# caiyuanhao1998/Open-DiffusionGS

Measured on AMD Instinct MI355X. Metric: novel-view renders/sec (DiT step + GS raster) at 256^2, higher is better.
Workload: dtype bf16; 1 GPU; obj-256 sampling step (BASELINE.json configs[2]): DGSDenoiser.forward = DiT image_to_gaussians (width 1024, 24 blocks, L=4098, bf16 MFMA, fp32 accumulate) + 4 fp32 rasterizations of P=262146 Gaussians at 256^2 per sample; random-init weights; batch_per_gpu=1, views=4, resolution=256, gaussians=262146, parallelism=dp1

## Files before the change

### include/dgs_dit.h

```cpp
#ifndef DGS_DIT_H_
#define DGS_DIT_H_

#include <stddef.h>
#include <stdint.h>

#include "dgs_raster.h"

#ifdef __cplusplus
extern "C" {
#endif

typedef enum DgsGemmEpilogue {
    DGS_EPI_BF16 = 0,
    DGS_EPI_GELU_BF16 = 1,
    DGS_EPI_GATE_RESIDUAL = 2,
    DGS_EPI_F32 = 3,
    DGS_EPI_QKV = 4,
    DGS_EPI_DGELU_BF16 = 5
} DgsGemmEpilogue;

typedef enum DgsGemmAlgo {
    DGS_GEMM_AUTO = 0,
    DGS_GEMM_SIMPLE128 = 1,
    DGS_GEMM_SLICED = 4,
    DGS_GEMM_QUAD = 5,
    DGS_GEMM_SLICED128 = 6
} DgsGemmAlgo;

typedef struct DgsDitGemmArgs {
    int32_t M, N, K;
    const uint16_t* A;
    int32_t lda;
    const uint16_t* W;
    int32_t ldw;
    const float* bias;
    int32_t epilogue;
    void* out;
    int32_t ldo;
    const float* gate;
    int32_t gate_stride;
    int32_t rows_per_batch;
    uint16_t* vt;
    const float* resid;
    void* aux;
    int32_t k_per_batch;
    int64_t a_batch_stride, w_batch_stride;
    int32_t algo;
    int32_t valid_rows;
    float q_scale;
    float* splitk_ws;
} DgsDitGemmArgs;

size_t dgs_dit_gemm_splitk_bytes(int32_t M, int32_t N, int32_t K, int32_t k_per_batch);

typedef struct DgsDitAttentionArgs {
    int32_t B, heads, L, lpad;
    const uint16_t* qk;
    const uint16_t* vt;
    uint16_t* out;
    float scale;
    int32_t ld_qk;
    int32_t k_offset;
    int64_t vt_batch_stride;
    float* lse2;
    int32_t q_prescaled;
    void* tail_ws;
    size_t tail_ws_bytes;
    int32_t tail_mode;
} DgsDitAttentionArgs;

size_t dgs_dit_attention_tail_bytes(int32_t B, int32_t heads, int32_t L);

typedef struct DgsDitAttentionBackwardArgs {
    int32_t B, heads, L, lpad;
    const uint16_t* qkv;
    const uint16_t* qkvT;
    const uint16_t* o;
    const uint16_t* dO;
    const uint16_t* dOT;
    const float* lse2;
    float* D;
    uint16_t* dqkv;
    float scale;
    uint16_t* dqkvT;
    float* bias_part;
} DgsDitAttentionBackwardArgs;
int32_t dgs_dit_attention_backward_slots(int32_t L);

typedef struct DgsDitLayerNormArgs {
    int32_t rows, width;
    const float* x;
    const float* weight;
    const float* shift;
    const float* scale;
    int32_t mod_stride;
    int32_t rows_per_batch;
    float eps;
    void* out;
    int32_t out_f32;
} DgsDitLayerNormArgs;

typedef struct DgsDitLayerNormBackwardArgs {
    int32_t rows, width;
    const float* x;
    const void* dh;
    int32_t dh_f32;
    const float* weight;
    const float* scale;
    int32_t mod_stride, rows_per_batch;
    float eps;
    const float* dx_in;
    float* dx_out;
    float *dshift, *dscale, *dweight;
    void* scratch;
    size_t scratch_bytes;
} DgsDitLayerNormBackwardArgs;

typedef struct DgsDitRowLinearBackwardArgs {
    int32_t M, N, K;
    const float* x;
    int32_t silu_input;
    const uint16_t* W;
    const float* dy;
    float *dW, *db, *dx;
    void* scratch;
    size_t scratch_bytes;
} DgsDitRowLinearBackwardArgs;

typedef struct DgsDitGateMulArgs {
    int32_t B, rows, width;
    const float* dx;
    const uint16_t* y;
    const float* gate;
    int32_t gate_stride;
    uint16_t *dy, *dyT;
    float* dgate;
    float* dbias;
    void* scratch;
    size_t scratch_bytes;
} DgsDitGateMulArgs;

typedef struct DgsDitRowLinearArgs {
    int32_t M, N, K;
    const float* x;
    int32_t silu_input;
    const uint16_t* W;
    const float* bias;
    int32_t silu_output;
    float* out;
} DgsDitRowLinearArgs;

typedef struct DgsDitLayerWeights {
    const uint16_t *qkv_w, *proj_w, *fc1_w, *fc2_w;
    const float *qkv_b, *proj_b, *fc1_b, *fc2_b;
} DgsDitLayerWeights;

typedef struct DgsDitModel {
    int32_t width, heads, layers, patch, in_channels, n_gaussians, gs_channels;
    int32_t scene;
    int32_t relative_plk;
    float range_near, range_far;
    const uint16_t* t_w0; const float* t_b0;
    const uint16_t* t_w1; const float* t_b1;
    const uint16_t* tok_w;
    const float* pos_emb;
    const float* in_ln_w;
    const DgsDitLayerWeights* layer;
    const uint16_t* ada_w; const float* ada_b;
    const float* up_ln_w;  const uint16_t* up_w;
    const float* dec_ln_w; const uint16_t* dec_w;
} DgsDitModel;

typedef struct DgsDitForwardArgs {
    int32_t B, V, H, W;
    const float* images;
    const float* ray_o;
    const float* ray_d;
    const int64_t* t;
    void* workspace;
    size_t workspace_bytes;
    float* xyz;
    float* features;
    float* scaling;
    float* rotation;
    float* opacity;
    float* aligned_xyz;
    float* tokens;
    void** prof_events;
    int32_t prof_kind;
    int32_t prof_capacity;
    int32_t* prof_count;
    int32_t train_recompute;
} DgsDitForwardArgs;

typedef struct DgsDitLayerWeightsT {
    const uint16_t *qkv_wT, *proj_wT, *fc1_wT, *fc2_wT;
} DgsDitLayerWeightsT;

typedef struct DgsDitModelT {
    const DgsDitLayerWeightsT* layer;
    const uint16_t* dec_wT;
} DgsDitModelT;

typedef struct DgsDitLayerGrads {
    float *qkv_w, *proj_w, *fc1_w, *fc2_w, *qkv_b, *proj_b, *fc1_b, *fc2_b;
    float *ada_w, *ada_b;
} DgsDitLayerGrads;

typedef struct DgsDitGrads {
    float *t_w0, *t_b0, *t_w1, *t_b1, *tok_w, *pos_emb, *in_ln_w;
    const DgsDitLayerGrads* layer;
    float *head_ada_w, *head_ada_b;
    float *up_ln_w, *up_w, *dec_ln_w, *dec_w;
} DgsDitGrads;

typedef struct DgsDitBackwardArgs {
    int32_t B, V, H, W;
    const float* ray_d;
    void* saved;        size_t saved_bytes;
    void* workspace;    size_t workspace_bytes;
    const float *dxyz, *dfeatures, *dscaling, *drotation, *dopacity;
    int32_t recompute;
    void (*block_done)(void* user, int32_t stage);
    void* block_user;
} DgsDitBackwardArgs;

size_t dgs_dit_saved_bytes(const DgsDitModel* m, int32_t B, int32_t V, int32_t H, int32_t W, int32_t recompute);
size_t dgs_dit_backward_workspace_bytes(const DgsDitModel* m, int32_t B, int32_t V, int32_t H, int32_t W);
int dgs_dit_forward_train(const DgsDitModel* m, const DgsDitForwardArgs* a, void* saved, size_t saved_bytes, dgs_stream_t stream);
int dgs_dit_backward(const DgsDitModel* m, const DgsDitModelT* mt, const DgsDitGrads* grads, const DgsDitBackwardArgs* a,
                     dgs_stream_t stream);

int dgs_dit_gemm(const DgsDitGemmArgs* a, dgs_stream_t stream);
int32_t dgs_dit_gemm_sliced_tile(const DgsDitGemmArgs* a);
int dgs_dit_attention(const DgsDitAttentionArgs* a, dgs_stream_t stream);
int dgs_dit_attention_backward(const DgsDitAttentionBackwardArgs* a, dgs_stream_t stream);
int dgs_dit_layernorm(const DgsDitLayerNormArgs* a, dgs_stream_t stream);
int dgs_dit_layernorm_gemm(const DgsDitLayerNormArgs* ln, const DgsDitGemmArgs* g, dgs_stream_t stream);
int32_t dgs_dit_layernorm_gemm_shares_rows(const DgsDitLayerNormArgs* ln, const DgsDitGemmArgs* g);
int dgs_dit_layernorm_backward(const DgsDitLayerNormBackwardArgs* a, dgs_stream_t stream);
int dgs_dit_rowlinear_backward(const DgsDitRowLinearBackwardArgs* a, dgs_stream_t stream);
int dgs_dit_gate_mul(const DgsDitGateMulArgs* a, dgs_stream_t stream);
size_t dgs_dit_layernorm_backward_scratch_bytes(int32_t rows, int32_t width, int32_t rows_per_batch);
size_t dgs_dit_rowlinear_backward_scratch_bytes(int32_t M, int32_t N, int32_t K);
size_t dgs_dit_gate_mul_scratch_bytes(int32_t B, int32_t rows, int32_t width);
int dgs_dit_rowlinear(const DgsDitRowLinearArgs* a, dgs_stream_t stream);

typedef struct DgsDitRunBlocksArgs {
    int32_t B, L, V;
    int32_t first, last;
    const float* tokens_in;
    const float* cvec;
    float* tokens_out;
    void* workspace;
    size_t workspace_bytes;
} DgsDitRunBlocksArgs;
size_t dgs_dit_workspace_bytes_for_tokens(const DgsDitModel* m, int32_t B, int32_t L);
int dgs_dit_run_blocks(const DgsDitModel* m, const DgsDitRunBlocksArgs* a, dgs_stream_t stream);

int dgs_debug_poison_lds(dgs_stream_t stream);

int dgs_debug_clock_probe(int64_t* out, int32_t microseconds, dgs_stream_t stream);

int32_t dgs_dit_lpad(int32_t L);
size_t dgs_dit_workspace_bytes(const DgsDitModel* m, int32_t B, int32_t V, int32_t H, int32_t W);
int dgs_dit_forward(const DgsDitModel* m, const DgsDitForwardArgs* a, dgs_stream_t stream);

#ifdef __cplusplus
}
#endif
#endif
```

### open-diffusiongs_amd/csrc/dit_gemm.hip

```cpp
#include <stdlib.h>

#include "dit_common.h"
#include "dgs_dit.h"
#include "dit_gemm_epilogue.h"

namespace dgs {

constexpr int BM = 128, BK = 64;
constexpr int TILE_BYTES = BM * BK * 2;

struct GemmParams {
    int M, N, K, lda, ldw, ldo, gate_stride, rows_per_batch, valid_rows, tiles_n, ntiles, tiles_m, map_mode;
    int rows_ps, full_rows;
    int ntail, tail_row0;
    int k_per_batch;
    long long a_batch_stride, w_batch_stride;
    const bf16_t* A;
    const bf16_t* W;
    const float* bias;
    void* out;
    const float* gate;
    const float* resid;
    bf16_t* vt;
    void* aux;
    float q_scale;
};

__device__ __forceinline__ float gelu_tanh(float x) {
    const float u = 0.7978845608028654f * (x + 0.044715f * x * x * x);
    return x / (1.0f + __expf(-2.0f * u));
}

__device__ __forceinline__ float dgelu_tanh(float x) {
    const float u = 0.7978845608028654f * (x + 0.044715f * x * x * x);
    const float sg = 1.0f / (1.0f + __expf(-2.0f * u));
    return sg + x * sg * (1.0f - sg) * (2.0f * 0.7978845608028654f) * (1.0f + 3.0f * 0.044715f * x * x);
}

template <int ROWS>
__device__ __forceinline__ void stage_tile(const bf16_t* g, int ld, int row0, int k0, char* lds_tile, int wave, int lane) {
#pragma unroll
    for (int q = 0; q < ROWS / 32; ++q) {
        const int piece = wave * (ROWS / 32) + q;
        const int row = piece * 8 + (lane >> 3);
        const int slot = lane & 7;
        const int chunk = slot ^ ((row >> 1) & 7);
        const bf16_t* src = g + (size_t)(row0 + row) * ld + k0 + chunk * 8;
        glds16(src, lds_tile + piece * 1024);
    }
}

template <int NI, int MI>
__device__ __forceinline__ void mma_tile(const char* la, const char* lb, int fhalf, int swz, f32x16 (&acc)[2][NI]) {
    bf16x8 a[2][MI], b[2][NI];
    auto read = [&](int ks, int h) {
        const int off = ((2 * ks + fhalf) ^ swz) << 4;
#pragma unroll
        for (int i = 0; i < MI; ++i) a[h][i] = *reinterpret_cast<const bf16x8*>(la + i * 32 * 128 + off);
#pragma unroll
        for (int j = 0; j < NI; ++j) b[h][j] = *reinterpret_cast<const bf16x8*>(lb + j * 32 * 128 + off);
    };
    read(0, 0);
#pragma unroll
    for (int ks = 0; ks < 4; ++ks) {
        const int h = ks & 1;
#pragma unroll
        for (int i = 0; i < MI; ++i)
#pragma unroll
            for (int j = 0; j < NI; ++j) {
                acc[i][j] = __builtin_amdgcn_mfma_f32_32x32x16_bf16(a[h][i], b[h][j], acc[i][j], 0, 0, 0);
                if (i == 0 && j == 0 && ks < 3) read(ks + 1, h ^ 1);
                sched_fence();
            }
    }
}

template <int BN, int NI, int MI, bool ONE_BATCH>
__device__ __forceinline__ void main_loop(const GemmParams& p, char* lds, int m0, int n0, int wave, int lane, int wm, int wn,
                                          f32x16 (&acc)[2][NI]) {
    constexpr int STAGE_BYTES = TILE_BYTES + BN * BK * 2;
    const int nk = p.K / BK;
    const int spb = p.k_per_batch / BK;
    stage_tile<BM>(p.A, p.lda, m0, 0, lds, wave, lane);
    stage_tile<BN>(p.W, p.ldw, n0, 0, lds + TILE_BYTES, wave, lane);
    __syncthreads();
    const int frow = lane & 31, fhalf = lane >> 5;
    const int swz = (frow >> 1) & 7;
    for (int t = 0; t < nk; ++t) {
        char* cur = lds + (t & 1) * STAGE_BYTES;
        if (t + 1 < nk) {
            char* nxt = lds + ((t + 1) & 1) * STAGE_BYTES;
            const int bb = ONE_BATCH ? 0 : (t + 1) / spb, kk = ((t + 1) - bb * spb) * BK;
            stage_tile<BM>(p.A + bb * p.a_batch_stride, p.lda, m0, kk, nxt, wave, lane);
            stage_tile<BN>(p.W + bb * p.w_batch_stride, p.ldw, n0, kk, nxt + TILE_BYTES, wave, lane);
        }
        if (MI > 0) {
            const char* la = cur + (wm * 64 + frow) * 128;
            const char* lb = cur + TILE_BYTES + (wn * (BN / 2) + frow) * 128;
            mma_tile<NI, (MI > 0 ? MI : 1)>(la, lb, fhalf, swz, acc);
        }
        __syncthreads();
    }
}

template <int EPI>
__device__ __forceinline__ void gemv_tail_rows(const GemmParams& p, char* lds, int item, int wave, int lane) {
    constexpr int CPI = 8;
    const int nblk = p.N / CPI, b = item / nblk, tn0 = (item - b * nblk) * CPI;
    const int tm0 = b * p.rows_per_batch + p.tail_row0;
    const int kw = p.K / 4, k_lo = wave * kw;
    const int nch = (kw + 511) / 512;
    const bool on0 = lane * 8 < kw, on1 = 512 + lane * 8 < kw;
    const bf16_t* a_row0 = p.A + (size_t)tm0 * p.lda + k_lo + lane * 8;
    const bf16_t* w_col0 = p.W + (size_t)tn0 * p.ldw + k_lo + lane * 8;
    const uint4 zero = make_uint4(0u, 0u, 0u, 0u);
    const int er = lane / CPI, ec = lane - er * CPI;
    const bool finisher = wave == 0 && lane < 2 * CPI && p.tail_row0 + er < p.valid_rows;
    TailOperands ops{0.f, 0.f, 0.f};
    if (finisher) ops = tail_prefetch<EPI>(p, tm0 + er, tn0 + ec);
    uint4 a[2][2], w[CPI][2];
#pragma unroll
    for (int ch = 0; ch < 2; ++ch) {
        const bool on = ch == 0 ? on0 : (on1 && nch > 1);
#pragma unroll
        for (int r = 0; r < 2; ++r) a[r][ch] = on ? *reinterpret_cast<const uint4*>(a_row0 + (size_t)r * p.lda + ch * 512) : zero;
#pragma unroll
        for (int c = 0; c < CPI; ++c) w[c][ch] = on ? *reinterpret_cast<const uint4*>(w_col0 + (size_t)c * p.ldw + ch * 512) : zero;
    }
    float* const part = reinterpret_cast<float*>(lds);
#pragma unroll
    for (int c = 0; c < CPI; ++c) {
        float s0 = dot8_bf16(a[0][0], w[c][0], 0.f), s1 = dot8_bf16(a[1][0], w[c][0], 0.f);
        s0 = dot8_bf16(a[0][1], w[c][1], s0); s1 = dot8_bf16(a[1][1], w[c][1], s1);
        s0 = wave_sum_lane63(s0); s1 = wave_sum_lane63(s1);
        if (lane == 63) { part[(wave * 2 + 0) * CPI + c] = s0; part[(wave * 2 + 1) * CPI + c] = s1; }
    }
    __syncthreads();
    if (finisher) {
        const int r = er, c = ec;
        const float v = (part[(0 * 2 + r) * CPI + c] + part[(1 * 2 + r) * CPI + c]) + (part[(2 * 2 + r) * CPI + c] + part[(3 * 2 + r) * CPI + c]);
        tail_store<EPI>(p, tm0 + r, tn0 + c, v, ops);
    }
}

template <int EPI, int BN>
__global__ __launch_bounds__(256) void gemm_bf16_kernel(GemmParams p) {
    constexpr int NI = BN / 64;
    constexpr int STAGE_BYTES = TILE_BYTES + BN * BK * 2;
    __shared__ __attribute__((aligned(16))) char lds[2 * STAGE_BYTES];
    const int tid = threadIdx.x, lane = tid & 63;
    const int wave = __builtin_amdgcn_readfirstlane(tid >> 6);
    const int wm = wave >> 1, wn = wave & 1;
    if ((int)blockIdx.x >= p.ntiles) {
        gemv_tail_rows<EPI>(p, lds, (int)blockIdx.x - p.ntiles, wave, lane);
        return;
    }
    const int logical = xcd_remap((int)blockIdx.x, p.ntiles);
    int tn, tr;
    if (p.map_mode >= 2) {
        const int gsz = p.map_mode * p.tiles_n, grp = logical / gsz, in = logical - grp * gsz;
        const int first = grp * p.map_mode, gm = min(p.tiles_m - first, p.map_mode);
        tr = first + in % gm;
        tn = in / gm;
    } else {
        tn = p.map_mode ? logical / p.tiles_m : logical % p.tiles_n;
        tr = p.map_mode ? logical % p.tiles_m : logical / p.tiles_n;
    }
    const int tm = (tr / p.full_rows) * p.rows_ps + tr % p.full_rows;
    const int m0 = tm * BM, n0 = tn * BN;
    const int mrow = m0 - (m0 / p.rows_per_batch) * p.rows_per_batch + wm * 64;
    const bool live0 = mrow < p.valid_rows, live1 = mrow + 32 < p.valid_rows;

    f32x16 acc[2][NI];
#pragma unroll
    for (int i = 0; i < 2; ++i)
#pragma unroll
        for (int j = 0; j < NI; ++j)
#pragma unroll
            for (int r = 0; r < 16; ++r) acc[i][j][r] = 0.0f;

    if (p.k_per_batch == p.K) {
        if (live1) main_loop<BN, NI, 2, true>(p, lds, m0, n0, wave, lane, wm, wn, acc);
        else if (live0) main_loop<BN, NI, 1, true>(p, lds, m0, n0, wave, lane, wm, wn, acc);
        else main_loop<BN, NI, 0, true>(p, lds, m0, n0, wave, lane, wm, wn, acc);
    } else {
        if (live1) main_loop<BN, NI, 2, false>(p, lds, m0, n0, wave, lane, wm, wn, acc);
        else if (live0) main_loop<BN, NI, 1, false>(p, lds, m0, n0, wave, lane, wm, wn, acc);
        else main_loop<BN, NI, 0, false>(p, lds, m0, n0, wave, lane, wm, wn, acc);
    }
    const int fhalf = lane >> 5;

    if (epi_staged<EPI>(p)) {
        char* patch = lds + wave * epi_strip_bytes(NI);
        if constexpr (EPI == DGS_EPI_GATE_RESIDUAL) {
            float4 pre[2][4 * NI];
#pragma unroll
            for (int mi = 0; mi < 2; ++mi)
                if (mi == 0 ? live0 : live1) residual_prefetch<NI>(p, m0 + wm * 64 + mi * 32, n0 + wn * (BN / 2), lane, pre[mi]);
#pragma unroll
            for (int mi = 0; mi < 2; ++mi)
                if (mi == 0 ? live0 : live1) store_strip<EPI, NI>(p, acc[mi], m0 + wm * 64 + mi * 32, n0 + wn * (BN / 2), lane, patch, pre[mi]);
            return;
        }
#pragma unroll
        for (int mi = 0; mi < 2; ++mi)
            if (mi == 0 ? live0 : live1) store_strip<EPI, NI>(p, acc[mi], m0 + wm * 64 + mi * 32, n0 + wn * (BN / 2), lane, patch);
        return;
    }

#pragma unroll
    for (int ni = 0; ni < NI; ++ni) {
        const int n = n0 + wn * (BN / 2) + ni * 32 + (lane & 31);
        const float bias = p.bias ? p.bias[n] : 0.0f;
        const float qs = (EPI == DGS_EPI_QKV && n < p.N / 3) ? p.q_scale : 1.0f;
#pragma unroll
        for (int mi = 0; mi < 2; ++mi) {
            if (!(mi == 0 ? live0 : live1)) continue;
            const int mbase = m0 + wm * 64 + mi * 32 + 4 * fhalf;
            const int b = mbase / p.rows_per_batch;
            const bool qkv_v = EPI == DGS_EPI_QKV && n >= (p.N / 3) * 2;
            bf16_t* tdst = nullptr;
            if (EPI == DGS_EPI_QKV) {
                if (qkv_v) tdst = p.vt + ((size_t)b * (p.N / 3) + (n - (p.N / 3) * 2)) * p.rows_per_batch + (mbase - b * p.rows_per_batch);
            } else if ((EPI == DGS_EPI_BF16 || EPI == DGS_EPI_GELU_BF16 || EPI == DGS_EPI_DGELU_BF16) && p.vt) {
                tdst = p.vt + ((size_t)b * p.N + n) * p.rows_per_batch + (mbase - b * p.rows_per_batch);
            }
            float gate = 0.0f;
            if (EPI == DGS_EPI_GATE_RESIDUAL) gate = p.gate[(size_t)b * p.gate_stride + n];
#pragma unroll
            for (int g = 0; g < 4; ++g) {
                float o4[4];
#pragma unroll
                for (int q = 0; q < 4; ++q) {
                    const int m = mbase + q + 8 * g;
                    const float v = EPI == DGS_EPI_QKV ? (acc[mi][ni][4 * g + q] + bias) * qs : acc[mi][ni][4 * g + q] + bias;
                    const size_t o = (size_t)m * p.ldo + n;
                    if (EPI == DGS_EPI_BF16) {
                        o4[q] = v;
                        reinterpret_cast<bf16_t*>(p.out)[o] = (bf16_t)f2bf_fast(v);
                    } else if (EPI == DGS_EPI_QKV) {
                        o4[q] = v;
                        if (!qkv_v) reinterpret_cast<bf16_t*>(p.out)[o] = (bf16_t)f2bf_fast(v);
                    } else if (EPI == DGS_EPI_GELU_BF16) {
                        o4[q] = gelu_tanh(v);
                        reinterpret_cast<bf16_t*>(p.out)[o] = (bf16_t)f2bf_fast(o4[q]);
                        if (p.aux) reinterpret_cast<bf16_t*>(p.aux)[o] = (bf16_t)f2bf_fast(v);
                    } else if (EPI == DGS_EPI_DGELU_BF16) {
                        o4[q] = v * dgelu_tanh(bf2f(reinterpret_cast<const bf16_t*>(p.aux)[o]));
                        reinterpret_cast<bf16_t*>(p.out)[o] = (bf16_t)f2bf_fast(o4[q]);
                    } else if (EPI == DGS_EPI_GATE_RESIDUAL) {
                        reinterpret_cast<float*>(p.out)[o] = p.resid[o] + gate * v;
                        if (p.aux) reinterpret_cast<bf16_t*>(p.aux)[o] = (bf16_t)f2bf_fast(v);
                    } else {
                        reinterpret_cast<float*>(p.out)[o] = v;
                    }
                }
                if (tdst) *reinterpret_cast<uint2*>(tdst + 8 * g) = make_uint2(pack_bf2(o4[0], o4[1]), pack_bf2(o4[2], o4[3]));
            }
        }
    }
}

int sliced_gemm_tile(int M, int N, int K, int epilogue, int k_per_batch, int rows_per_batch, int valid_rows);
int launch_sliced_gemm(const DgsDitGemmArgs* a, int bn, int rows_per_batch, int valid_rows, hipStream_t st, bool quad, bool rows_external);
bool sliced_rows_are_gemv(int K, int N, int valid_rows);
bool sliced128_eligible(int M, int N, int K, int epilogue, int k_per_batch, int rows_per_batch);
int splitk_plan(int M, int N, int K, int k_per_batch, int* splits_per_batch);
int launch_splitk_gemm(const DgsDitGemmArgs* a, int k_per_batch, hipStream_t st);

}

using namespace dgs;

template <int EPI>
static void launch_gemm(const GemmParams& p0, int bn, hipStream_t st) {
    GemmParams p = p0;
    p.tiles_n = p.N / bn;
    p.rows_ps = p.rows_per_batch / BM;
    p.full_rows = (p.valid_rows + BM - 1) / BM;
    const int last_live = p.valid_rows - (p.full_rows - 1) * BM;
    static const int no_tail = getenv("DGS_GEMM_NO_GEMV_TAIL") ? atoi(getenv("DGS_GEMM_NO_GEMV_TAIL")) : 0;
    p.ntail = 0; p.tail_row0 = 0;
    if (!no_tail && p.full_rows > 1 && last_live <= 2 && p.K % 512 == 0 && p.K <= 4096 && p.k_per_batch == p.K && p.N % 8 == 0 &&
        !(EPI == DGS_EPI_QKV)) {
        --p.full_rows;
        p.tail_row0 = p.full_rows * BM;
        p.ntail = (p.M / p.rows_per_batch) * (p.N / 8);
    }
    p.tiles_m = (p.M / p.rows_per_batch) * p.full_rows;
    p.ntiles = p.tiles_m * p.tiles_n;
    static const int map_env = getenv("DGS_GEMM_MAP") ? atoi(getenv("DGS_GEMM_MAP")) : 0;
    p.map_mode = map_env;
    if (bn == 128) hipLaunchKernelGGL((gemm_bf16_kernel<EPI, 128>), dim3(p.ntail + p.ntiles), dim3(256), 0, st, p);
    else hipLaunchKernelGGL((gemm_bf16_kernel<EPI, 64>), dim3(p.ntail + p.ntiles), dim3(256), 0, st, p);
}

static int gemm_dispatch(const DgsDitGemmArgs* a, dgs_stream_t stream, int mode) {
    if (!a || a->M <= 0 || a->N <= 0 || a->K <= 0 || a->M % BM || a->N % 64 || a->K % BK) return DGS_ERR_INVALID_ARGUMENT;
    if (!a->A || !a->W || !a->out || (a->lda & 7) || (a->ldw & 7)) return DGS_ERR_INVALID_ARGUMENT;
    const int kpb = a->k_per_batch > 0 ? a->k_per_batch : a->K;
    if (kpb % BK || a->K % kpb || a->lda < kpb || a->ldw < kpb) return DGS_ERR_INVALID_ARGUMENT;
    if (a->epilogue == DGS_EPI_GATE_RESIDUAL && (!a->gate || a->rows_per_batch <= 0)) return DGS_ERR_INVALID_ARGUMENT;
    if (a->epilogue == DGS_EPI_QKV && (!a->vt || a->N % 3 || (a->N / 3) % 128)) return DGS_ERR_INVALID_ARGUMENT;
    if (a->epilogue == DGS_EPI_DGELU_BF16 && !a->aux) return DGS_ERR_INVALID_ARGUMENT;
    if ((a->vt || a->epilogue == DGS_EPI_QKV) && a->rows_per_batch <= 0) return DGS_ERR_INVALID_ARGUMENT;
    if (a->rows_per_batch > 0 && (a->rows_per_batch % BM || a->M % a->rows_per_batch)) return DGS_ERR_INVALID_ARGUMENT;
    GemmParams p;
    p.M = a->M; p.N = a->N; p.K = a->K; p.lda = a->lda; p.ldw = a->ldw; p.ldo = a->ldo;
    p.gate_stride = a->gate_stride; p.rows_per_batch = a->rows_per_batch > 0 ? a->rows_per_batch : a->M;
    p.valid_rows = (a->valid_rows > 0 && a->valid_rows < p.rows_per_batch) ? a->valid_rows : p.rows_per_batch;
    p.k_per_batch = kpb; p.a_batch_stride = a->a_batch_stride; p.w_batch_stride = a->w_batch_stride;
    p.A = a->A; p.W = a->W; p.bias = a->bias; p.out = a->out; p.gate = a->gate; p.vt = a->vt; p.aux = a->aux;
    p.q_scale = a->q_scale != 0.0f ? a->q_scale : 1.0f;
    p.resid = a->resid ? a->resid : static_cast<const float*>(a->out);
    hipStream_t st0 = static_cast<hipStream_t>(stream);
    static const int env_algo = getenv("DGS_GEMM_ALGO") ? atoi(getenv("DGS_GEMM_ALGO")) : 0;
    const int algo = a->algo ? a->algo : env_algo;
    if (mode == 0 && (algo == DGS_GEMM_AUTO || algo == DGS_GEMM_SLICED) && a->splitk_ws && a->epilogue == DGS_EPI_F32 && !a->bias && a->ldo % 4 == 0 &&
        p.rows_per_batch == a->M && p.valid_rows == a->M) {
        int spb = 0;
        if (splitk_plan(a->M, a->N, a->K, kpb, &spb)) return launch_splitk_gemm(a, kpb, st0);
    }
    const int sbn_auto = algo == DGS_GEMM_AUTO ? sliced_gemm_tile(a->M, a->N, a->K, a->epilogue, kpb, p.rows_per_batch, p.valid_rows) : 0;
    const bool auto_sliced = sbn_auto != 0 && (a->M > 8192 || ((sbn_auto == 256 || sbn_auto == 192) && (a->epilogue == DGS_EPI_QKV ||
                                                                                  (a->epilogue == DGS_EPI_GELU_BF16 && a->N >= 4096))));
    if (algo == DGS_GEMM_SLICED || algo == DGS_GEMM_QUAD || auto_sliced) {
        const int sbn = sliced_gemm_tile(a->M, a->N, a->K, a->epilogue, kpb, p.rows_per_batch, p.valid_rows);
        if (mode == 3) return sbn;
        if (mode == 2) return sbn && sliced_rows_are_gemv(a->K, a->N, p.valid_rows) && p.valid_rows < p.rows_per_batch ? 1 : 0;
        if (sbn) return launch_sliced_gemm(a, sbn, p.rows_per_batch, p.valid_rows, st0, algo == DGS_GEMM_QUAD, mode == 1);
    }
    if (mode == 2 || mode == 3) return 0;
    if (mode == 1) return DGS_ERR_INVALID_ARGUMENT;
    static const int no_s128 = getenv("DGS_GEMM_NO_SLICED128") ? atoi(getenv("DGS_GEMM_NO_SLICED128")) : 0;
    static const int s128_mink = getenv("DGS_GEMM_S128_MINK") ? atoi(getenv("DGS_GEMM_S128_MINK")) : 1024;
    const bool few_tiles = (a->M / BM) * (a->N / 128) < 512 && a->N % 128 == 0;
    if ((algo == DGS_GEMM_SLICED128 || (algo == DGS_GEMM_AUTO && few_tiles && !no_s128 && a->K >= s128_mink)) &&
        sliced128_eligible(a->M, a->N, a->K, a->epilogue, kpb, p.rows_per_batch))
        return launch_sliced_gemm(a, -128, p.rows_per_batch, p.valid_rows, st0, false, false);
    if (a->epilogue == DGS_EPI_QKV && a->N % 128) return DGS_ERR_INVALID_ARGUMENT;
    static const int env_bn = getenv("DGS_GEMM_BN") ? atoi(getenv("DGS_GEMM_BN")) : 0;
    int bn = (a->N % 128 || ((a->M / BM) * (a->N / 128) < 512 && a->epilogue != DGS_EPI_QKV)) ? 64 : 128;
    if (env_bn == 128 && a->N % 128 == 0) bn = 128;
    if (env_bn == 64) bn = 64;
    hipStream_t st = static_cast<hipStream_t>(stream);
    switch (a->epilogue) {
        case DGS_EPI_BF16: launch_gemm<DGS_EPI_BF16>(p, bn, st); break;
        case DGS_EPI_GELU_BF16: launch_gemm<DGS_EPI_GELU_BF16>(p, bn, st); break;
        case DGS_EPI_GATE_RESIDUAL: launch_gemm<DGS_EPI_GATE_RESIDUAL>(p, bn, st); break;
        case DGS_EPI_F32: launch_gemm<DGS_EPI_F32>(p, bn, st); break;
        case DGS_EPI_QKV: launch_gemm<DGS_EPI_QKV>(p, 128, st); break;
        case DGS_EPI_DGELU_BF16: launch_gemm<DGS_EPI_DGELU_BF16>(p, bn, st); break;
        default: return DGS_ERR_INVALID_ARGUMENT;
    }
    return hipGetLastError() == hipSuccess ? DGS_OK : DGS_ERR_DEVICE;
}

extern "C" int dgs_dit_gemm(const DgsDitGemmArgs* a, dgs_stream_t stream) { return gemm_dispatch(a, stream, 0); }
extern "C" int32_t dgs_dit_gemm_sliced_tile(const DgsDitGemmArgs* a) { const int w = gemm_dispatch(a, nullptr, 3); return w > 0 ? w : 0; }

namespace dgs {
bool gemm_leaves_rows_out(const DgsDitGemmArgs* a) { return gemm_dispatch(a, nullptr, 2) == 1; }
int launch_gemm_external_rows(const DgsDitGemmArgs* a, dgs_stream_t stream) { return gemm_dispatch(a, stream, 1); }
}

extern "C" size_t dgs_dit_gemm_splitk_bytes(int32_t M, int32_t N, int32_t K, int32_t k_per_batch) {
    int spb = 0;
    const int nsplit = dgs::splitk_plan(M, N, K, k_per_batch > 0 ? k_per_batch : K, &spb);
    return (size_t)nsplit * M * N * sizeof(float);
}
```

### open-diffusiongs_amd/csrc/dit_gemm_deep.hip

```cpp
#include <stdio.h>
#include <stdlib.h>
#include <type_traits>

#include "dit_common.h"
#include "dgs_dit.h"
#include "dit_gemm_epilogue.h"

namespace dgs {

struct DeepParams {
    int M, N, K, lda, ldw, ldo, gate_stride, rows_per_batch, valid_rows, tiles_n, ntiles, dbg;
    int rows_ps, full_rows, tail_rows, nfull_items;
    int ntail, tail_mode;
    int tail_wgs;
    int map2d;
    int rows_external;
    int nsplit, splits_per_batch;
    long long a_batch_stride, w_batch_stride, out_split_stride;
    const bf16_t* A;
    const bf16_t* W;
    const float* bias;
    void* out;
    const float* gate;
    const float* resid;
    bf16_t* vt;
    void* aux;
    float q_scale;
};

__device__ __forceinline__ float gelu_tanh_d(float x) {
    const float u = 0.7978845608028654f * (x + 0.044715f * x * x * x);
    return x / (1.0f + __expf(-2.0f * u));
}
__device__ __forceinline__ float dgelu_tanh_d(float x) {
    const float u = 0.7978845608028654f * (x + 0.044715f * x * x * x);
    const float sg = 1.0f / (1.0f + __expf(-2.0f * u));
    return sg + x * sg * (1.0f - sg) * (2.0f * 0.7978845608028654f) * (1.0f + 3.0f * 0.044715f * x * x);
}

template <int BK>
__device__ __forceinline__ int slab_off(int r, int c) {
    return BK == 64 ? r * 128 + ((c ^ ((r >> 1) & 7)) << 4) : r * 64 + ((c ^ ((r >> 2) & 3)) << 4);
}

template <int EPI, int NI>
__device__ __forceinline__ void store_block(const DeepParams& p, const f32x16 (&acc)[NI], int mbase, int nbase, int lane) {
    const int b = mbase / p.rows_per_batch;
#pragma unroll
    for (int ni = 0; ni < NI; ++ni) {
        const int n = nbase + ni * 32 + (lane & 31);
        const float bias = p.bias ? p.bias[n] : 0.0f;
        const float qs = (EPI == DGS_EPI_QKV && n < p.N / 3) ? p.q_scale : 1.0f;
        const bool qkv_v = EPI == DGS_EPI_QKV && n >= (p.N / 3) * 2;
        bf16_t* tdst = nullptr;
        if (EPI == DGS_EPI_QKV) {
            if (qkv_v) tdst = p.vt + ((size_t)b * (p.N / 3) + (n - (p.N / 3) * 2)) * p.rows_per_batch + (mbase - b * p.rows_per_batch);
        } else if ((EPI == DGS_EPI_BF16 || EPI == DGS_EPI_GELU_BF16 || EPI == DGS_EPI_DGELU_BF16) && p.vt) {
            tdst = p.vt + ((size_t)b * p.N + n) * p.rows_per_batch + (mbase - b * p.rows_per_batch);
        }
        float gate = 0.0f;
        if (EPI == DGS_EPI_GATE_RESIDUAL) gate = p.gate[(size_t)b * p.gate_stride + n];
#pragma unroll
        for (int g = 0; g < 4; ++g) {
            float o4[4];
#pragma unroll
            for (int q = 0; q < 4; ++q) {
                const int m = mbase + q + 8 * g;
                const float v = EPI == DGS_EPI_QKV ? (acc[ni][4 * g + q] + bias) * qs : acc[ni][4 * g + q] + bias;
                const size_t o = (size_t)m * p.ldo + n;
                if (EPI == DGS_EPI_BF16) {
                    o4[q] = v;
                    reinterpret_cast<bf16_t*>(p.out)[o] = (bf16_t)f2bf_fast(v);
                } else if (EPI == DGS_EPI_QKV) {
                    o4[q] = v;
                    if (!qkv_v) reinterpret_cast<bf16_t*>(p.out)[o] = (bf16_t)f2bf_fast(v);
                } else if (EPI == DGS_EPI_GELU_BF16) {
                    o4[q] = gelu_tanh_d(v);
                    reinterpret_cast<bf16_t*>(p.out)[o] = (bf16_t)f2bf_fast(o4[q]);
                    if (p.aux) reinterpret_cast<bf16_t*>(p.aux)[o] = (bf16_t)f2bf_fast(v);
                } else if (EPI == DGS_EPI_DGELU_BF16) {
                    o4[q] = v * dgelu_tanh_d(bf2f(reinterpret_cast<const bf16_t*>(p.aux)[o]));
                    reinterpret_cast<bf16_t*>(p.out)[o] = (bf16_t)f2bf_fast(o4[q]);
                } else if (EPI == DGS_EPI_GATE_RESIDUAL) {
                    reinterpret_cast<float*>(p.out)[o] = p.resid[o] + gate * v;
                    if (p.aux) reinterpret_cast<bf16_t*>(p.aux)[o] = (bf16_t)f2bf_fast(v);
                } else {
                    reinterpret_cast<float*>(p.out)[o] = v;
                }
            }
            if (tdst) *reinterpret_cast<uint2*>(tdst + 8 * g) = make_uint2(pack_bf2(o4[0], o4[1]), pack_bf2(o4[2], o4[3]));
        }
    }
}

template <int I> struct SIC { static constexpr int value = I; };
template <int I, int N, class F> __device__ __forceinline__ void sliced_for(F&& f) {
    if constexpr (I < N) { f(SIC<I>{}); sliced_for<I + 1, N>(f); }
}

__device__ long long dgs_gemm_dbg[16];
__device__ unsigned dgs_gemm_tl[1024][4];

template <int EPI, int BN, int NW, int EXP = 0, int BM = 256>
__global__ __launch_bounds__(NW == 8 ? 512 : 256) void gemm_sliced_kernel(DeepParams p) {
    constexpr int KW = (BM == 128 && NW == 8) ? 2 : 1, MW = NW / KW;
    constexpr int BK = 32, NS = (BM == 128 && KW == 1) ? 8 : 4;
    constexpr int WMB = BM / (16 * MW), WROWS = 32 * WMB;
    constexpr int WN = BN / 2, NI = WN / 32;
    constexpr int A_BYTES = BM * BK * 2, W_BYTES = BN * BK * 2, SUB = A_BYTES + W_BYTES, STAGE = KW * SUB;
    constexpr int W_PIECES = KW * W_BYTES / 1024, GW = (W_PIECES + NW - 1) / NW, DUP = NW * GW - W_PIECES;
    constexpr int G = KW * A_BYTES / 1024 / NW + GW;
    static_assert(KW == 1 || (A_BYTES / 1024 == NW && W_BYTES / 1024 == NW && WMB == 2 && NI == 2), "K groups: piece q of an operand is slab q's, one per wave");
    constexpr int NF = WMB + NI, MF = WMB * NI;
    static_assert(NW == 8 || BN == 256 || (BM == 128 && BN == 128), "4 waves: 256 x 256 tiles (128 x 128 per wave) or 128 x 128 tiles (64 x 64)");
    static_assert(DUP == 0 || (DUP < NW && GW >= 1 && KW == 1), "a doubled piece only in the last W round");
    static_assert(WMB * NI >= G, "one DMA piece behind each MFMA of the spread half");
    DGS_DYNAMIC_LDS(lds);
    const int dbg = kInstrumented ? p.dbg : 0;
    const long long dbg_k0 = dbg == 1 ? cycle_stamp() : 0;
    const long long dbg_w0 = dbg == 1 ? wall_stamp() : 0;
    const int tid = threadIdx.x, lane = tid & 63;
    const int wave = __builtin_amdgcn_readfirstlane(tid >> 6);
    const int wq = KW > 1 ? wave % MW : wave, kg = KW > 1 ? wave / MW : 0;
    const int wm = wq >> 1, wn = wq & 1;
    const int frow = lane & 31, fhalf = lane >> 5;
    const int bid = (int)blockIdx.x;
    const bf16_t* const A_all = p.A;
    const bf16_t* const W_all = p.W;
    const int K_all = p.K;
    auto side_jobs = [&](const int first, const int stride) {
        if (p.tail_mode == 2) {
            const int KS = min(NW, K_all / 512), CS = NW / KS, CPI = 8 * CS;
            const int nblk = p.N / CPI;
            const int kq = wave % KS, cq = wave / KS;
            const int kw = K_all / KS, k_lo = kq * kw;
            const bool two = kw > 512;
            float* const part = reinterpret_cast<float*>(lds + (NS - 1) * STAGE);
            const uint4 zero = make_uint4(0u, 0u, 0u, 0u);
            for (int j = first; j < p.ntail; j += stride) {
                const int blk = j % nblk, trr = j / nblk;
                const int tm0 = ((trr / p.tail_rows) * p.rows_ps + p.full_rows + trr % p.tail_rows) * BM, tn0 = blk * CPI + cq * 8;
                const bf16_t* a_row0 = A_all + (size_t)tm0 * p.lda + k_lo + lane * 8;
                const bf16_t* w_col0 = W_all + (size_t)tn0 * p.ldw + k_lo + lane * 8;
                const int er = tid / CPI, ec = tid - er * CPI;
                const int erow = tm0 + er;
                const bool finisher = tid < 2 * CPI && erow - (erow / p.rows_per_batch) * p.rows_per_batch < p.valid_rows;
                TailOperands ops{0.f, 0.f, 0.f};
                if (finisher) ops = tail_prefetch<EPI>(p, erow, blk * CPI + ec);
                uint4 a[2][2], w[8][2];
#pragma unroll
                for (int ch = 0; ch < 2; ++ch) {
                    const bool on = ch == 0 || two;
#pragma unroll
                    for (int r = 0; r < 2; ++r) a[r][ch] = on ? *reinterpret_cast<const uint4*>(a_row0 + (size_t)r * p.lda + ch * 512) : zero;
#pragma unroll
                    for (int c = 0; c < 8; ++c) w[c][ch] = on ? *reinterpret_cast<const uint4*>(w_col0 + (size_t)c * p.ldw + ch * 512) : zero;
                }
#pragma unroll
                for (int c = 0; c < 8; ++c) {
                    float s0 = dot8_bf16(a[0][0], w[c][0], 0.f), s1 = dot8_bf16(a[1][0], w[c][0], 0.f);
                    s0 = dot8_bf16(a[0][1], w[c][1], s0); s1 = dot8_bf16(a[1][1], w[c][1], s1);
                    s0 = wave_sum_lane63(s0); s1 = wave_sum_lane63(s1);
                    if (lane == 63) { part[(kq * 2 + 0) * CPI + cq * 8 + c] = s0; part[(kq * 2 + 1) * CPI + cq * 8 + c] = s1; }
                }
                __syncthreads();
                if (finisher) {
                    float v = 0.f;
                    for (int q = 0; q < KS; ++q) v += part[(q * 2 + er) * CPI + ec];
                    tail_store<EPI>(p, erow, blk * CPI + ec, v, ops);
                }
                __syncthreads();
            }
            return;
        }
        for (int j = p.nsplit > 1 ? p.ntail : first; j < p.ntail; j += stride) {
            constexpr int CBW = BN == 256 ? 1 : 2, KQ = NW / CBW, TPC = BN / (32 * CBW);
            const int sub = j % TPC, ttn = (j / TPC) % p.tiles_n, trr = j / (TPC * p.tiles_n);
            const int tm0 = ((trr / p.tail_rows) * p.rows_ps + p.full_rows + trr % p.tail_rows) * BM, tn0 = ttn * BN + sub * 32 * CBW;
            const int cbl = wave % CBW, kq = wave / CBW, kper = K_all / KQ;
            const bf16_t* arow = A_all + (size_t)(tm0 + frow) * p.lda + kq * kper + fhalf * 8;
            const bf16_t* wrow = W_all + (size_t)(tn0 + cbl * 32 + frow) * p.ldw + kq * kper + fhalf * 8;
            f32x16 acc1[1];
#pragma unroll
            for (int r = 0; r < 16; ++r) acc1[0][r] = 0.f;
            if (kper % 256 == 0)
                for (int k = 0; k < kper; k += 256) direct_block_mfma<16>(arow + k, wrow + k, acc1[0]);
            else
                for (int k = 0; k < kper; k += 128) direct_block_mfma<8>(arow + k, wrow + k, acc1[0]);
            float* red = reinterpret_cast<float*>(lds + (NS - 1) * STAGE);
            if (kq > 0)
#pragma unroll
                for (int r = 0; r < 16; ++r) red[((kq - 1) * CBW + cbl) * 1024 + r * 64 + lane] = acc1[0][r];
            __syncthreads();
            if (kq == 0) {
#pragma unroll
                for (int q = 1; q < KQ; ++q)
#pragma unroll
                    for (int r = 0; r < 16; ++r) acc1[0][r] += red[((q - 1) * CBW + cbl) * 1024 + r * 64 + lane];
                store_block<EPI, 1>(p, acc1, tm0 + 4 * fhalf, tn0 + cbl * 32, lane);
            }
            __syncthreads();
        }
    };
    if (p.nfull_items == 0) { side_jobs(bid, (int)gridDim.x); return; }
    if (p.tail_wgs > 0 && bid >= p.nfull_items) { side_jobs(bid - p.nfull_items, p.tail_wgs); return; }
    int tile;
    if (p.nsplit > 1) {
        const int all = xcd_remap(bid, p.nfull_items * p.nsplit);
        const int sp = all / p.nfull_items, b = sp / p.splits_per_batch, part = sp % p.splits_per_batch;
        tile = all - sp * p.nfull_items;
        const int units = p.K / 128, u0 = part * units / p.splits_per_batch, u1 = (part + 1) * units / p.splits_per_batch;
        p.A += (size_t)b * p.a_batch_stride + u0 * 128;
        p.W += (size_t)b * p.w_batch_stride + u0 * 128;
        p.out = static_cast<float*>(p.out) + (size_t)sp * p.out_split_stride;
        p.K = (u1 - u0) * 128;
    } else if (p.map2d) {
        const int xcd = bid & 7, slot = bid >> 3, rows_all = p.nfull_items / p.tiles_n;
        const int rper = rows_all >> 2, cper = p.tiles_n >> 1;
        tile = ((xcd >> 1) * rper + slot / cper) * p.tiles_n + (xcd & 1) * cper + slot % cper;
    } else {
        tile = xcd_remap(bid, p.nfull_items);
    }
    const int tn = tile % p.tiles_n, rr = tile / p.tiles_n;
    const int m0 = ((rr / p.full_rows) * p.rows_ps + rr % p.full_rows) * BM, n0 = tn * BN;
    f32x16 acc[WMB][NI];
#pragma unroll
    for (int i = 0; i < WMB; ++i)
#pragma unroll
        for (int j = 0; j < NI; ++j)
#pragma unroll
            for (int r = 0; r < 16; ++r) acc[i][j][r] = 0.0f;
    int foff[2][NF];
#pragma unroll
    for (int ks = 0; ks < 2; ++ks)
#pragma unroll
        for (int f = 0; f < NF; ++f)
            foff[ks][f] = kg * SUB + (f < WMB ? slab_off<BK>(wm * WROWS + 32 * f + frow, 2 * ks + fhalf) : A_BYTES + slab_off<BK>(wn * WN + 32 * (f - WMB) + frow, 2 * ks + fhalf));
    auto frag = [&](int slot, int ks, int f) { return *reinterpret_cast<const bf16x8*>(lds + slot * STAGE + foff[ks][f]); };
    const int nk = p.K / (BK * KW);
    constexpr int GA = KW * A_BYTES / 1024 / NW;
    constexpr int RPI = 1024 / (2 * BK), CPR = BK / 8;
    char* const lds_mine = lds + wave * 1024;
    const uint32_t lds_wave = lds_address(lds) + (uint32_t)wave * 1024u;
    const char* sb_a = reinterpret_cast<const char*>(p.A + (size_t)m0 * p.lda);
    const char* sb_w = reinterpret_cast<const char*>(p.W + (size_t)n0 * p.ldw);
    uint32_t vo_a[GA], vo_w[G - GA];
    const int back = (DUP > 0 && wave + NW * (GW - 1) >= W_PIECES) ? DUP : 0;
    {
        const int r0 = lane / CPR, chunk = (lane % CPR) ^ (BK == 64 ? (r0 >> 1) & 7 : (r0 >> 2) & 3);
        if constexpr (KW > 1) {
#pragma unroll
            for (int q = 0; q < GA; ++q) vo_a[q] = (uint32_t)(((wave * RPI + r0) * p.lda + chunk * 8 + q * BK) * 2);
#pragma unroll
            for (int q = 0; q < G - GA; ++q) vo_w[q] = (uint32_t)(((wave * RPI + r0) * p.ldw + chunk * 8 + q * BK) * 2);
        } else {
#pragma unroll
            for (int q = 0; q < GA; ++q) vo_a[q] = (uint32_t)((((wave + NW * q) * RPI + r0) * p.lda + chunk * 8) * 2);
#pragma unroll
            for (int q = 0; q < G - GA; ++q) vo_w[q] = (uint32_t)((((wave + NW * q - (q == GW - 1 ? back : 0)) * RPI + r0) * p.ldw + chunk * 8) * 2);
        }
    }
    char* const lds_mine_last = lds_mine - back * 1024;
    const uint32_t lds_wave_last = lds_wave - (uint32_t)back * 1024u;
    auto dma_piece = [&](auto slotc, auto qc) {
        constexpr int slot = decltype(slotc)::value, q = decltype(qc)::value;
        if constexpr (KW > 1 && q < GA) lds_dma_scalar<slot * STAGE + q * SUB>(sb_a, vo_a[q], lds_wave, lds_mine);
        else if constexpr (KW > 1) lds_dma_scalar<slot * STAGE + (q - GA) * SUB + A_BYTES>(sb_w, vo_w[q - GA], lds_wave, lds_mine);
        else if constexpr (q < GA) lds_dma_scalar<slot * STAGE + NW * q * 1024>(sb_a, vo_a[q], lds_wave, lds_mine);
        else if constexpr (DUP > 0 && q == G - 1) lds_dma_scalar<slot * STAGE + A_BYTES + NW * (q - GA) * 1024>(sb_w, vo_w[q - GA], lds_wave_last, lds_mine_last);
        else lds_dma_scalar<slot * STAGE + A_BYTES + NW * (q - GA) * 1024>(sb_w, vo_w[q - GA], lds_wave, lds_mine);
        if constexpr (q == G - 1) { sb_a += 2 * BK * KW; sb_w += 2 * BK * KW; }
    };
    auto stage_next = [&](auto slotc) { sliced_for<0, G>([&](auto qc) { dma_piece(slotc, qc); }); };
    const bool has_side_job = NS > 4 && p.tail_wgs == 0 && bid < p.ntail && p.nsplit == 1;
    sliced_for<0, 2>([&](auto sc) { stage_next(sc); });
    if (!has_side_job) sliced_for<2, NS - 1>([&](auto sc) { stage_next(sc); });
    if (p.tail_wgs == 0) side_jobs(bid, (int)gridDim.x);
    if (has_side_job) sliced_for<2, NS - 1>([&](auto sc) { stage_next(sc); });
    wait_vmcnt<(NS - 3) * G>();
    raw_barrier();
    bf16x8 fr[2][NF];
#pragma unroll
    for (int f = 0; f < NF; ++f) fr[0][f] = frag(0, 0, f);

    long long dbg_wait = 0, dbg_bar = 0;
    constexpr bool SPREAD = NW == 4;
    constexpr bool PREFETCH_RESID = EPI == DGS_EPI_GATE_RESIDUAL && BM == 128;
    constexpr int PRE_BLOCKS = KW > 1 ? 1 : WMB;
    constexpr int PRE_LOADS = PREFETCH_RESID ? PRE_BLOCKS * (NI / 2) * 8 : 0;
    float4 pre[PREFETCH_RESID ? PRE_BLOCKS * (NI / 2) : 1][8];
    auto iteration = [&](int t, auto slot_tag, auto refill_tag, auto pre_tag, auto left_tag, auto dbg_tag) {
        constexpr bool DBG = decltype(dbg_tag)::value;
        constexpr int slot = decltype(slot_tag)::value;
        constexpr int PRE_N = decltype(pre_tag)::value;
        constexpr bool refill = decltype(refill_tag)::value;
        if constexpr (refill && !SPREAD && EXP != 1) stage_next(SIC<(slot + NS - 1) % NS>{});
        sliced_for<0, 2 * MF>([&](auto jc) {
            constexpr int J = decltype(jc)::value, ks = J / MF, i = (J % MF) / NI, j = J % NI;
            acc[i][j] = __builtin_amdgcn_mfma_f32_32x32x16_bf16(fr[ks][i], fr[ks][WMB + j], acc[i][j], 0, 0, 0);
            sched_fence();
            constexpr int f = J % MF;
            if constexpr (f < NF && EXP != 2) fr[ks ^ 1][f] = frag(ks == 0 ? slot : (slot + 1) % NS, ks ^ 1, f);
            if constexpr (SPREAD && refill && ks == 0 && f >= MF - G && EXP != 1) {
                constexpr int q = f - (MF - G);
                dma_piece(SIC<(slot + NS - 1) % NS>{}, SIC<q>{});
            }
            sched_fence();
        });
        if constexpr (PRE_N > 0 && refill) {
            if constexpr (KW > 1) {
#pragma unroll
                for (int j = 0; j < NI; j += 2) residual_prefetch<2>(p, m0 + wm * WROWS + 32 * kg, n0 + wn * WN + 32 * j, lane, pre[j / 2]);
            } else {
#pragma unroll
                for (int i = 0; i < WMB; ++i)
#pragma unroll
                    for (int j = 0; j < NI; j += 2) residual_prefetch<2>(p, m0 + wm * WROWS + 32 * i, n0 + wn * WN + 32 * j, lane, pre[i * (NI / 2) + j / 2]);
            }
        }
        long long w0 = 0;
        if constexpr (DBG) w0 = cycle_stamp();
        if constexpr (PRE_N > 0) {
            constexpr int left = decltype(left_tag)::value;
            wait_vmcnt<left * G + PRE_N>();
        } else if constexpr (refill) wait_vmcnt<(NS - 3) * G>();
        else wait_vmcnt<0>();
        long long w1 = 0;
        if constexpr (DBG) w1 = cycle_stamp();
        raw_barrier();
        if constexpr (DBG) { dbg_wait += w1 - w0; dbg_bar += cycle_stamp() - w1; }
        (void)t;
    };
    const long long dbg_t0 = dbg == 1 ? cycle_stamp() : 0;
    const long long dbg_w1 = dbg == 1 ? wall_stamp() : 0;
    auto k_loop = [&](auto dbg_tag) {
        for (int t = 0; t < nk - NS; t += NS)
            sliced_for<0, NS>([&](auto sc) { iteration(t + decltype(sc)::value, sc, std::true_type{}, SIC<0>{}, SIC<0>{}, dbg_tag); });
        sliced_for<0, NS>([&](auto sc) {
            constexpr int S = decltype(sc)::value;
            iteration(nk - NS + S, sc, std::integral_constant<bool, S == 0>{}, SIC<PRE_LOADS>{}, SIC<(NS - S - 3 > 0 ? NS - S - 3 : 0)>{}, dbg_tag);
        });
    };
    if constexpr (kInstrumented) {
        if (dbg == 1) k_loop(std::true_type{});
        else k_loop(std::false_type{});
    } else {
        k_loop(std::false_type{});
    }
    const long long dbg_t1 = dbg == 1 ? cycle_stamp() : 0;
    const long long dbg_w2 = dbg == 1 ? wall_stamp() : 0;
    if constexpr (KW > 1) {
        float* const xch = reinterpret_cast<float*>(lds);
        auto region = [&](int owner) { return xch + ((wq * 2 + owner) * NI * 16) * 64 + lane; };
        auto give = [&](const f32x16 (&blk)[NI], float* dst) {
#pragma unroll
            for (int j = 0; j < NI; ++j)
#pragma unroll
                for (int r = 0; r < 16; ++r) dst[(j * 16 + r) * 64] = blk[j][r];
        };
        auto take = [&](f32x16 (&blk)[NI], const float* src) {
#pragma unroll
            for (int j = 0; j < NI; ++j)
#pragma unroll
                for (int r = 0; r < 16; ++r) blk[j][r] += src[(j * 16 + r) * 64];
        };
        if (kg == 0) give(acc[1], region(1)); else give(acc[0], region(0));
        __syncthreads();
        if (kg == 0) take(acc[0], region(0)); else take(acc[1], region(1));
        __syncthreads();
        char* patch = lds + wave * epi_strip_bytes(2);
        const int mb = m0 + wm * WROWS + 32 * kg, nb = n0 + wn * WN;
        if (kg == 0) {
            if constexpr (PREFETCH_RESID) store_strip<EPI, 2>(p, &acc[0][0], mb, nb, lane, patch, pre[0]);
            else store_strip<EPI, 2>(p, &acc[0][0], mb, nb, lane, patch);
        } else {
            if constexpr (PREFETCH_RESID) store_strip<EPI, 2>(p, &acc[1][0], mb, nb, lane, patch, pre[0]);
            else store_strip<EPI, 2>(p, &acc[1][0], mb, nb, lane, patch);
        }
    } else
    if (epi_staged<EPI>(p)) {
        char* patch = lds + wave * epi_strip_bytes(2);
        if constexpr (NI % 2 == 1) {
            const int nb = n0 + wn * WN, v0 = (p.N / 3) * 2;
            const bool straddles = EPI == DGS_EPI_QKV && nb < v0 && nb + 64 > v0;
#pragma unroll
            for (int i = 0; i < WMB; ++i) {
                const int mb = m0 + wm * WROWS + 32 * i;
                if (straddles) { store_strip<EPI, 1>(p, &acc[i][0], mb, nb, lane, patch); store_strip<EPI, 1>(p, &acc[i][1], mb, nb + 32, lane, patch); }
                else store_strip<EPI, 2>(p, &acc[i][0], mb, nb, lane, patch);
                store_strip<EPI, 1>(p, &acc[i][NI - 1], mb, nb + 32 * (NI - 1), lane, patch);
            }
        } else
#pragma unroll
        for (int i = 0; i < WMB; ++i)
#pragma unroll
            for (int j = 0; j < NI; j += 2) {
                if constexpr (PREFETCH_RESID) store_strip<EPI, 2>(p, &acc[i][j], m0 + wm * WROWS + 32 * i, n0 + wn * WN + 32 * j, lane, patch, pre[i * (NI / 2) + j / 2]);
                else store_strip<EPI, 2>(p, &acc[i][j], m0 + wm * WROWS + 32 * i, n0 + wn * WN + 32 * j, lane, patch);
            }
    } else {
#pragma unroll
        for (int i = 0; i < WMB; ++i) store_block<EPI, NI>(p, acc[i], m0 + wm * WROWS + 32 * i + 4 * fhalf, n0 + wn * WN, lane);
    }
    if constexpr (kInstrumented) if (dbg == 1) {
        wait_vmcnt<0>();
        if (tid == 0 && bid < 1024) {
            dgs_gemm_tl[bid][0] = (unsigned)dbg_w0; dgs_gemm_tl[bid][1] = (unsigned)dbg_w1; dgs_gemm_tl[bid][2] = (unsigned)dbg_w2;
            dgs_gemm_tl[bid][3] = (unsigned)wall_stamp();
        }
        if (tid == 0) {
            atomicMax(reinterpret_cast<unsigned long long*>(&dgs_gemm_dbg[6]), (unsigned long long)(cycle_stamp() - dbg_k0));
            atomicMax(reinterpret_cast<unsigned long long*>(&dgs_gemm_dbg[7]), (unsigned long long)dbg_wait);
            atomicMin(reinterpret_cast<unsigned long long*>(&dgs_gemm_dbg[8]), (unsigned long long)dbg_k0);
            atomicMax(reinterpret_cast<unsigned long long*>(&dgs_gemm_dbg[9]), (unsigned long long)cycle_stamp());
        }
        if (blockIdx.x == 0 && tid == 0) {
            dgs_gemm_dbg[0] = dbg_t1 - dbg_t0; dgs_gemm_dbg[1] = dbg_wait; dgs_gemm_dbg[2] = dbg_bar; dgs_gemm_dbg[3] = nk;
            dgs_gemm_dbg[4] = dbg_t0 - dbg_k0; dgs_gemm_dbg[5] = cycle_stamp() - dbg_t1;
            dgs_gemm_dbg[10] = cycle_stamp() - dbg_k0; dgs_gemm_dbg[11] = wall_stamp() - dbg_w0;
        }
    }
}

template <int EPI, int BN, int NW = 8, int BM = 256>
static int launch_sliced(DeepParams p, hipStream_t st) {
    constexpr int LDS = (BM == 128 ? 8 : 4) * (BM * 32 * 2 + BN * 32 * 2);
    p.tiles_n = p.N / BN;
    p.rows_ps = p.rows_per_batch / BM;
    p.full_rows = 0; p.tail_rows = 0;
    const int last_live = p.valid_rows - (p.valid_rows - 1) / BM * BM;
    const bool gemv_ok = last_live <= 2 && p.K >= 512 && p.K <= 4096 && (p.K & (p.K - 1)) == 0 && p.N % 64 == 0;
    const bool mfma_ok = p.K % (NW / (BN == 256 ? 1 : 2) * 128) == 0;
    for (int i = 0; i < p.rows_ps; ++i) {
        const int live = (p.valid_rows - i * BM + 31) / 32;
        if (live > 1 || (live == 1 && !gemv_ok && !mfma_ok)) ++p.full_rows; else if (live == 1) ++p.tail_rows;
    }
    if (p.rows_external) {
        if (!gemv_ok || p.nsplit > 1) return DGS_ERR_INVALID_ARGUMENT;
        p.tail_rows = 0;
    }
    const int samples = p.M / p.rows_per_batch;
    p.nfull_items = samples * p.full_rows * p.tiles_n;
    p.tail_mode = gemv_ok ? 2 : 1;
    const int gemv_ks = NW < p.K / 512 ? NW : p.K / 512, gemv_cpi = 8 * (NW / (gemv_ks > 0 ? gemv_ks : 1));
    p.ntail = samples * p.tail_rows * (gemv_ok ? p.N / gemv_cpi : p.tiles_n * (BN / (BN == 256 ? 32 : 64)));
    p.ntiles = p.nfull_items ? p.nfull_items : p.ntail;
    p.tail_wgs = 0;
    if (p.nsplit <= 1 && p.ntail > 0 && p.nfull_items > 0) {
        static const int ncu = compute_unit_count();
        const int idle = ncu - p.nfull_items;
        if (idle > 0) p.tail_wgs = idle < p.ntail ? idle : p.ntail;
        p.ntiles += p.tail_wgs;
    }
    if (p.nsplit > 1) {
        if (p.tail_rows || samples != 1) return DGS_ERR_INVALID_ARGUMENT;
        p.ntiles = p.nfull_items * p.nsplit;
    }
    static const int no_map2d = getenv("DGS_GEMM_NO_MAP2D") ? atoi(getenv("DGS_GEMM_NO_MAP2D")) : 0;
    const int rows_all = samples * p.full_rows;
    p.map2d = !no_map2d && BM == 256 && p.nsplit <= 1 && p.tail_wgs == 0 && rows_all % 4 == 0 && p.tiles_n % 2 == 0 && p.nfull_items % 8 == 0 &&
              p.nfull_items <= compute_unit_count_cached() ? 1 : 0;
    auto kern = gemm_sliced_kernel<EPI, BN, NW, 0, BM>;
    if constexpr (kInstrumented && EPI == DGS_EPI_F32 && BN == 256 && BM == 256) {
        static const int exp = getenv("DGS_GEMM_EXP") ? atoi(getenv("DGS_GEMM_EXP")) : 0;
        if (exp == 1) kern = gemm_sliced_kernel<EPI, BN, NW, 1>;
        if (exp == 2) kern = gemm_sliced_kernel<EPI, BN, NW, 2>;
        if (exp && hipFuncSetAttribute(reinterpret_cast<const void*>(kern), hipFuncAttributeMaxDynamicSharedMemorySize, LDS) != hipSuccess) return DGS_ERR_DEVICE;
    }
    static bool attr_set = false;
    if (!attr_set) {
        if (hipFuncSetAttribute(reinterpret_cast<const void*>(kern), hipFuncAttributeMaxDynamicSharedMemorySize, LDS) != hipSuccess) return DGS_ERR_DEVICE;
        attr_set = true;
    }
    static const int dbg = kInstrumented && getenv("DGS_GEMM_DBG") ? atoi(getenv("DGS_GEMM_DBG")) : 0;
    p.dbg = dbg;
#ifdef DGS_INSTRUMENT
    if (dbg == 1) {
        const long long z[4] = {0, 0, 0x7fffffffffffffffLL, 0};
        (void)hipStreamSynchronize(st);
        if (hipMemcpyToSymbol(HIP_SYMBOL(dgs_gemm_dbg), z, sizeof(z), 6 * sizeof(long long), hipMemcpyHostToDevice) != hipSuccess) fprintf(stderr, "[gemm dbg] reset failed\n");
    }
#endif
    hipLaunchKernelGGL(kern, dim3(p.ntiles), dim3(64 * NW), LDS, st, p);
#ifdef DGS_INSTRUMENT
    if (dbg == 1) {
        long long h[12];
        (void)hipStreamSynchronize(st);
        (void)hipMemcpyFromSymbol(h, HIP_SYMBOL(dgs_gemm_dbg), sizeof(h));
        {
            static unsigned tl[1024][4];
            (void)hipMemcpyFromSymbol(tl, HIP_SYMBOL(dgs_gemm_tl), sizeof(tl));
            const int n = p.ntiles < 1024 ? p.ntiles : 1024;
            unsigned t0 = 0xffffffffu;
            for (int i = 0; i < n; ++i) t0 = tl[i][0] < t0 ? tl[i][0] : t0;
            double acc[4] = {0, 0, 0, 0}, mn[4] = {1e9, 1e9, 1e9, 1e9}, mx[4] = {0, 0, 0, 0};
            const int nt = p.nfull_items < n ? p.nfull_items : n;
            for (int i = 0; i < nt; ++i)
                for (int k = 0; k < 4; ++k) { const double v = (tl[i][k] - t0) / 100.0; acc[k] += v; mn[k] = v < mn[k] ? v : mn[k]; mx[k] = v > mx[k] ? v : mx[k]; }
            fprintf(stderr, "[gemm timeline] %d tile workgroups (of %d), us since the first start: start %.2f/%.2f/%.2f  loop start %.2f/%.2f/%.2f  loop end %.2f/%.2f/%.2f  end %.2f/%.2f/%.2f (min/mean/max)\n",
                    nt, n, mn[0], acc[0] / nt, mx[0], mn[1], acc[1] / nt, mx[1], mn[2], acc[2] / nt, mx[2], mn[3], acc[3] / nt, mx[3]);
            double xe[8] = {0}, xl[8] = {0}; int xn[8] = {0};
            for (int i = 0; i < nt; ++i) { xe[i & 7] += (tl[i][3] - t0) / 100.0; xl[i & 7] += (tl[i][2] - tl[i][1]) / 100.0; ++xn[i & 7]; }
            fprintf(stderr, "[gemm timeline] by block id %% 8 (XCD): mean loop us / mean end us:");
            for (int x = 0; x < 8; ++x) fprintf(stderr, " %.2f/%.2f", xn[x] ? xl[x] / xn[x] : 0.0, xn[x] ? xe[x] / xn[x] : 0.0);
            double se = 0, s2 = 0;
            int c1 = 0, c2 = 0;
            for (int i = 0; i < nt; ++i) { if (p.tail_wgs == 0 && i < p.ntail) { se += (tl[i][1] - tl[i][0]) / 100.0; ++c1; } else { s2 += (tl[i][1] - tl[i][0]) / 100.0; ++c2; } }
            fprintf(stderr, "\n[gemm timeline] prologue us: %d workgroups with a side job %.2f, %d without %.2f\n", c1, c1 ? se / c1 : 0.0, c2, c2 ? s2 / c2 : 0.0);
        }
        fprintf(stderr, "[gemm dbg] M=%d N=%d K=%d BN=%d: prologue %lld, loop %lld cycles (%lld per slab), vmcnt wait %lld, barrier %lld, epilogue %lld | slowest wg %lld cycles, max vmcnt wait %lld per slab, workgroup 0: %lld cycles in %.2f us = %.0f MHz\n", p.M,
                p.N, p.K, BN, h[4], h[0], h[0] / h[3], h[1] / h[3], h[2] / h[3], h[5], h[6], h[7] / h[3], h[10], h[11] / 100.0, h[10] / (h[11] / 100.0));
    }
#endif
    return hipGetLastError() == hipSuccess ? DGS_OK : DGS_ERR_DEVICE;
}

int sliced_gemm_tile(int M, int N, int K, int epilogue, int k_per_batch, int rows_per_batch, int valid_rows) {
    if (k_per_batch != K || K % 128 || M % 256 || rows_per_batch % 256) return 0;
    if (epilogue == DGS_EPI_QKV && N % 3) return 0;
    int full_rows = 0;
    for (int i = 0; i < rows_per_batch / 256; ++i)
        if ((valid_rows - i * 256 + 31) / 32 > 1) ++full_rows;
    static const int no192 = getenv("DGS_GEMM_NO_BN192") ? atoi(getenv("DGS_GEMM_NO_BN192")) : 0;
    const int ncu = compute_unit_count_cached();
    const int rows_all = (M / rows_per_batch) * full_rows;
    const bool fills = rows_all * (N / 192) >= 160 || ncu < 160;
    if (!no192 && epilogue == DGS_EPI_QKV && N % 192 == 0 && N % 256 == 0 && rows_all * (N / 256) < ncu && rows_all * (N / 192) <= ncu && fills) return 192;
    if (N % 256 == 0 && rows_all * (N / 256) >= 160) return 256;
    return N % 128 ? 0 : 128;
}

bool sliced128_eligible(int M, int N, int K, int epilogue, int k_per_batch, int rows_per_batch) {
    return k_per_batch == K && K % 256 == 0 && M % 128 == 0 && rows_per_batch % 128 == 0 && N % 128 == 0 && epilogue != DGS_EPI_QKV;
}

bool sliced_rows_are_gemv(int K, int N, int valid_rows) {
    const int last_live = valid_rows - (valid_rows - 1) / 256 * 256;
    return last_live <= 2 && K >= 512 && K <= 4096 && (K & (K - 1)) == 0 && N % 64 == 0;
}

int launch_sliced_gemm(const DgsDitGemmArgs* a, int bn, int rows_per_batch, int valid_rows, hipStream_t st, bool quad, bool rows_external) {
    DeepParams p;
    p.rows_external = rows_external ? 1 : 0;
    p.M = a->M; p.N = a->N; p.K = a->K; p.lda = a->lda; p.ldw = a->ldw; p.ldo = a->ldo; p.gate_stride = a->gate_stride;
    p.rows_per_batch = rows_per_batch; p.valid_rows = valid_rows; p.dbg = 0; p.nsplit = 1; p.splits_per_batch = 1;
    p.a_batch_stride = p.w_batch_stride = p.out_split_stride = 0;
    p.A = a->A; p.W = a->W; p.bias = a->bias; p.out = a->out; p.gate = a->gate; p.vt = a->vt; p.aux = a->aux;
    p.q_scale = a->q_scale != 0.0f ? a->q_scale : 1.0f;
    p.resid = a->resid ? a->resid : static_cast<const float*>(a->out);
    static const int s128_nw4 = getenv("DGS_GEMM_S128_NW4") ? atoi(getenv("DGS_GEMM_S128_NW4")) : 0;
#define DGS_SLICED_CASE(E) case E: return bn == 256 ? (quad ? launch_sliced<E, 256, 4>(p, st) : launch_sliced<E, 256>(p, st)) : \
                                   bn == 128 ? launch_sliced<E, 128>(p, st) : s128_nw4 ? launch_sliced<E, 128, 4, 128>(p, st) : launch_sliced<E, 128, 8, 128>(p, st)
    if (bn == 192) return a->epilogue == DGS_EPI_QKV && !quad ? launch_sliced<DGS_EPI_QKV, 192>(p, st) : DGS_ERR_INVALID_ARGUMENT;
    switch (a->epilogue) {
        DGS_SLICED_CASE(DGS_EPI_BF16);
        DGS_SLICED_CASE(DGS_EPI_GELU_BF16);
        DGS_SLICED_CASE(DGS_EPI_GATE_RESIDUAL);
        DGS_SLICED_CASE(DGS_EPI_F32);
        DGS_SLICED_CASE(DGS_EPI_QKV);
        DGS_SLICED_CASE(DGS_EPI_DGELU_BF16);
        default: return DGS_ERR_INVALID_ARGUMENT;
    }
#undef DGS_SLICED_CASE
}

int splitk_plan(int M, int N, int K, int k_per_batch, int* splits_per_batch) {
    if (M <= 0 || N <= 0 || k_per_batch <= 0 || M % 256 || N % 256 || k_per_batch % 128 || K % k_per_batch) return 0;
    const int nb = K / k_per_batch, tiles = (M / 256) * (N / 256), units = k_per_batch / 128;
    if (nb > 8) return 0;
    const bool tiny = tiles <= 16;
    int s = 256 / (nb * tiles);
    if (s > 8 / nb) s = 8 / nb;
    if (s > units / (tiny ? 4 : 16)) s = units / (tiny ? 4 : 16);
    if (s < 1) s = 1;
    const char* e = getenv("DGS_SPLITK_MIN_ITEMS");
    if (nb * s < 2 || nb * s * tiles < (e ? atoi(e) : tiny ? 96 : 160)) return 0;
    *splits_per_batch = s;
    return nb * s;
}

__global__ __launch_bounds__(256) void splitk_reduce_kernel(const float* __restrict__ part, float* __restrict__ out, int nsplit, int N, int ldo,
                                                            size_t plane) {
    const size_t i = ((size_t)blockIdx.x * 256 + threadIdx.x) * 4;
    if (i >= plane) return;
    float4 acc = *reinterpret_cast<const float4*>(part + i);
    for (int s = 1; s < nsplit; ++s) {
        const float4 v = *reinterpret_cast<const float4*>(part + s * plane + i);
        acc.x += v.x; acc.y += v.y; acc.z += v.z; acc.w += v.w;
    }
    const size_t m = i / N, n = i - m * N;
    *reinterpret_cast<float4*>(out + m * ldo + n) = acc;
}

int launch_splitk_gemm(const DgsDitGemmArgs* a, int k_per_batch, hipStream_t st) {
    int spb = 1;
    const int nsplit = splitk_plan(a->M, a->N, a->K, k_per_batch, &spb);
    if (!nsplit || a->epilogue != DGS_EPI_F32 || a->bias || !a->splitk_ws || a->ldo % 4) return DGS_ERR_INVALID_ARGUMENT;
    DeepParams p;
    p.M = a->M; p.N = a->N; p.K = k_per_batch; p.lda = a->lda; p.ldw = a->ldw; p.ldo = a->N; p.gate_stride = 0;
    p.rows_per_batch = a->M; p.valid_rows = a->M; p.dbg = 0; p.nsplit = nsplit; p.splits_per_batch = spb;
    p.a_batch_stride = a->a_batch_stride; p.w_batch_stride = a->w_batch_stride; p.out_split_stride = (long long)a->M * a->N;
    p.A = a->A; p.W = a->W; p.bias = nullptr; p.out = a->splitk_ws; p.gate = nullptr; p.vt = nullptr; p.aux = nullptr; p.q_scale = 1.0f;
    p.resid = nullptr; p.rows_external = 0;
    const int rc = launch_sliced<DGS_EPI_F32, 256>(p, st);
    if (rc != DGS_OK) return rc;
    const size_t plane = (size_t)a->M * a->N;
    hipLaunchKernelGGL(splitk_reduce_kernel, dim3((unsigned)((plane / 4 + 255) / 256)), dim3(256), 0, st, a->splitk_ws, static_cast<float*>(a->out), nsplit,
                       a->N, a->ldo, plane);
    return hipGetLastError() == hipSuccess ? DGS_OK : DGS_ERR_DEVICE;
}

}
```

### open-diffusiongs_amd/csrc/dit_gemm_epilogue.h

```cpp
#pragma once
#include "dit_common.h"
#include "dgs_dit.h"

namespace dgs {

__device__ __forceinline__ float epi_gelu_tanh(float x) {
    const float t = x * __builtin_fmaf(x * x, -2.0f * 1.4426950408889634f * 0.7978845608028654f * 0.044715f, -2.0f * 1.4426950408889634f * 0.7978845608028654f);
    return x * hw_rcp(1.0f + hw_exp2(t));
}

__device__ __forceinline__ float epi_dgelu_tanh(float x) {
    const float t = x * __builtin_fmaf(x * x, -2.0f * 1.4426950408889634f * 0.7978845608028654f * 0.044715f, -2.0f * 1.4426950408889634f * 0.7978845608028654f);
    const float sg = hw_rcp(1.0f + hw_exp2(t));
    return sg + x * sg * (1.0f - sg) * (2.0f * 0.7978845608028654f) * __builtin_fmaf(x * x, 3.0f * 0.044715f, 1.0f);
}

template <int U>
__device__ __forceinline__ void direct_block_mfma(const bf16_t* arow, const bf16_t* wrow, f32x16& acc) {
    bf16x8 a[U], w[U];
#pragma unroll
    for (int u = 0; u < U; ++u) {
        a[u] = *reinterpret_cast<const bf16x8*>(arow + 16 * u);
        w[u] = *reinterpret_cast<const bf16x8*>(wrow + 16 * u);
    }
#pragma unroll
    for (int u = 0; u < U; ++u) acc = __builtin_amdgcn_mfma_f32_32x32x16_bf16(a[u], w[u], acc, 0, 0, 0);
}

__device__ __forceinline__ float dot8_bf16(const uint4& a, const uint4& b, float acc) {
#ifdef HIPEMU
    const unsigned x[4] = {a.x, a.y, a.z, a.w}, y[4] = {b.x, b.y, b.z, b.w};
    for (int i = 0; i < 4; ++i)
        acc += __uint_as_float(x[i] << 16) * __uint_as_float(y[i] << 16) + __uint_as_float(x[i] & 0xffff0000u) * __uint_as_float(y[i] & 0xffff0000u);
    return acc;
#else
    typedef __bf16 bf2_t __attribute__((ext_vector_type(2)));
    acc = __builtin_amdgcn_fdot2_f32_bf16(__builtin_bit_cast(bf2_t, a.x), __builtin_bit_cast(bf2_t, b.x), acc, false);
    acc = __builtin_amdgcn_fdot2_f32_bf16(__builtin_bit_cast(bf2_t, a.y), __builtin_bit_cast(bf2_t, b.y), acc, false);
    acc = __builtin_amdgcn_fdot2_f32_bf16(__builtin_bit_cast(bf2_t, a.z), __builtin_bit_cast(bf2_t, b.z), acc, false);
    return __builtin_amdgcn_fdot2_f32_bf16(__builtin_bit_cast(bf2_t, a.w), __builtin_bit_cast(bf2_t, b.w), acc, false);
#endif
}

__device__ __forceinline__ void store_token_octet(bf16_t* tdst, int g, int half, uint2 u0, uint2 u1) {
    half_swap(u0.x, u1.x);
    half_swap(u0.y, u1.y);
    *reinterpret_cast<uint4*>(tdst + 8 * (g + half)) = make_uint4(u0.x, u0.y, u1.x, u1.y);
}

constexpr int epi_strip_bytes(int nb) { return 32 * (32 * nb + 4) * 4; }


template <int EPI, class P>
__device__ __forceinline__ bool epi_staged(const P&) { return true; }

template <int NB, class P>
__device__ __forceinline__ void residual_prefetch(const P& p, int m0, int n0, int lane, float4 (&pre)[4 * NB]) {
    constexpr int C = 32 * NB, LPR = C / 4, RPI = 64 / LPR;
    const int rr = lane / LPR, cc = (lane % LPR) * 4;
#pragma unroll
    for (int it = 0; it < 32 / RPI; ++it) pre[it] = *reinterpret_cast<const float4*>(p.resid + (size_t)(m0 + it * RPI + rr) * p.ldo + n0 + cc);
}

template <int EPI, int NB, bool HAVE_PRE, class P>
__device__ __forceinline__ void store_strip_impl(const P& p, const f32x16* acc, int m0, int n0, int lane, char* patch, const float4 (&pre)[4 * NB]) {
    constexpr int C = 32 * NB, S = C + 4;
    const int c = lane & 31, half = lane >> 5;
    const int b = m0 / p.rows_per_batch;
    if (EPI == DGS_EPI_QKV && n0 >= (p.N / 3) * 2) {
#pragma unroll
        for (int blk = 0; blk < NB; ++blk) {
            const int n = n0 + 32 * blk + c;
            const float bias = p.bias ? p.bias[n] : 0.0f;
            bf16_t* tdst = p.vt + ((size_t)b * (p.N / 3) + (n - (p.N / 3) * 2)) * p.rows_per_batch + (m0 - b * p.rows_per_batch);
#pragma unroll
            for (int g = 0; g < 4; g += 2)
                store_token_octet(tdst, g, half,
                                  make_uint2(pack_bf2(acc[blk][4 * g] + bias, acc[blk][4 * g + 1] + bias), pack_bf2(acc[blk][4 * g + 2] + bias, acc[blk][4 * g + 3] + bias)),
                                  make_uint2(pack_bf2(acc[blk][4 * g + 4] + bias, acc[blk][4 * g + 5] + bias), pack_bf2(acc[blk][4 * g + 6] + bias, acc[blk][4 * g + 7] + bias)));
        }
        return;
    }
    float* st = reinterpret_cast<float*>(patch);
#pragma unroll
    for (int blk = 0; blk < NB; ++blk) {
        const int n = n0 + 32 * blk + c;
        const float bias = p.bias ? p.bias[n] : 0.0f;
        const float qs = (EPI == DGS_EPI_QKV && n < p.N / 3) ? p.q_scale : 1.0f;
#pragma unroll
        for (int r = 0; r < 16; ++r) {
            const int row = (r & 3) + 8 * (r >> 2) + 4 * half;
            st[row * S + 32 * blk + c] = EPI == DGS_EPI_QKV ? (acc[blk][r] + bias) * qs : acc[blk][r] + bias;
        }
    }
    __builtin_amdgcn_wave_barrier();
    if (EPI == DGS_EPI_F32 || EPI == DGS_EPI_GATE_RESIDUAL) {
        constexpr int LPR = C / 4, RPI = 64 / LPR;
        const int rr = lane / LPR, cc = (lane % LPR) * 4;
        float4 gate = make_float4(0.f, 0.f, 0.f, 0.f);
        if (EPI == DGS_EPI_GATE_RESIDUAL) gate = *reinterpret_cast<const float4*>(p.gate + (size_t)b * p.gate_stride + n0 + cc);
#pragma unroll
        for (int it = 0; it < 32 / RPI; ++it) {
            const int row = it * RPI + rr;
            const float4 v = *reinterpret_cast<const float4*>(st + row * S + cc);
            const size_t o = (size_t)(m0 + row) * p.ldo + n0 + cc;
            if (EPI == DGS_EPI_GATE_RESIDUAL) {
                float4 x;
                if constexpr (HAVE_PRE) x = pre[it]; else x = *reinterpret_cast<const float4*>(p.resid + o);
                *reinterpret_cast<float4*>(reinterpret_cast<float*>(p.out) + o) =
                    make_float4(x.x + gate.x * v.x, x.y + gate.y * v.y, x.z + gate.z * v.z, x.w + gate.w * v.w);
                if (p.aux) *reinterpret_cast<uint2*>(reinterpret_cast<bf16_t*>(p.aux) + o) = make_uint2(pack_bf2(v.x, v.y), pack_bf2(v.z, v.w));
            } else {
                *reinterpret_cast<float4*>(reinterpret_cast<float*>(p.out) + o) = v;
            }
        }
    } else {
        constexpr int LPR = C / 8, RPI = 64 / LPR;
        const int rr = lane / LPR, cc = (lane % LPR) * 8;
        const bool transposed = EPI != DGS_EPI_QKV && p.vt != nullptr;
#pragma unroll
        for (int it = 0; it < 32 / RPI; ++it) {
            const int row = it * RPI + rr;
            float4 v0 = *reinterpret_cast<const float4*>(st + row * S + cc), v1 = *reinterpret_cast<const float4*>(st + row * S + cc + 4);
            const size_t o = (size_t)(m0 + row) * p.ldo + n0 + cc;
            if (EPI == DGS_EPI_GELU_BF16) {
                if (p.aux) *reinterpret_cast<uint4*>(reinterpret_cast<bf16_t*>(p.aux) + o) =
                    make_uint4(pack_bf2(v0.x, v0.y), pack_bf2(v0.z, v0.w), pack_bf2(v1.x, v1.y), pack_bf2(v1.z, v1.w));
                v0 = make_float4(epi_gelu_tanh(v0.x), epi_gelu_tanh(v0.y), epi_gelu_tanh(v0.z), epi_gelu_tanh(v0.w));
                v1 = make_float4(epi_gelu_tanh(v1.x), epi_gelu_tanh(v1.y), epi_gelu_tanh(v1.z), epi_gelu_tanh(v1.w));
            } else if (EPI == DGS_EPI_DGELU_BF16) {
                const uint4 ax = *reinterpret_cast<const uint4*>(reinterpret_cast<const bf16_t*>(p.aux) + o);
                v0 = make_float4(v0.x * epi_dgelu_tanh(__uint_as_float(ax.x << 16)), v0.y * epi_dgelu_tanh(__uint_as_float(ax.x & 0xffff0000u)),
                                 v0.z * epi_dgelu_tanh(__uint_as_float(ax.y << 16)), v0.w * epi_dgelu_tanh(__uint_as_float(ax.y & 0xffff0000u)));
                v1 = make_float4(v1.x * epi_dgelu_tanh(__uint_as_float(ax.z << 16)), v1.y * epi_dgelu_tanh(__uint_as_float(ax.z & 0xffff0000u)),
                                 v1.z * epi_dgelu_tanh(__uint_as_float(ax.w << 16)), v1.w * epi_dgelu_tanh(__uint_as_float(ax.w & 0xffff0000u)));
            }
            *reinterpret_cast<uint4*>(reinterpret_cast<bf16_t*>(p.out) + o) =
                make_uint4(pack_bf2(v0.x, v0.y), pack_bf2(v0.z, v0.w), pack_bf2(v1.x, v1.y), pack_bf2(v1.z, v1.w));
            if (transposed && EPI != DGS_EPI_BF16) {
                *reinterpret_cast<float4*>(st + row * S + cc) = v0;
                *reinterpret_cast<float4*>(st + row * S + cc + 4) = v1;
            }
        }
        if (transposed) {
            __builtin_amdgcn_wave_barrier();
#pragma unroll
            for (int blk = 0; blk < NB; ++blk) {
                bf16_t* tdst = p.vt + ((size_t)b * p.N + n0 + 32 * blk + c) * p.rows_per_batch + (m0 - b * p.rows_per_batch);
#pragma unroll
                for (int g = 0; g < 4; g += 2) {
                    const float* src = st + (4 * half + 8 * g) * S + 32 * blk + c;
                    store_token_octet(tdst, g, half, make_uint2(pack_bf2(src[0], src[S]), pack_bf2(src[2 * S], src[3 * S])),
                                      make_uint2(pack_bf2(src[8 * S], src[9 * S]), pack_bf2(src[10 * S], src[11 * S])));
                }
            }
        }
    }
    __builtin_amdgcn_wave_barrier();
}

template <int EPI, int NB, class P>
__device__ __forceinline__ void store_strip(const P& p, const f32x16* acc, int m0, int n0, int lane, char* patch) {
    const float4 none[4 * NB] = {};
    store_strip_impl<EPI, NB, false>(p, acc, m0, n0, lane, patch, none);
}
template <int EPI, int NB, class P>
__device__ __forceinline__ void store_strip(const P& p, const f32x16* acc, int m0, int n0, int lane, char* patch, const float4 (&pre)[4 * NB]) {
    store_strip_impl<EPI, NB, true>(p, acc, m0, n0, lane, patch, pre);
}

struct TailOperands { float bias, resid, gate; };
template <int EPI, class P>
__device__ __forceinline__ TailOperands tail_prefetch(const P& p, int m, int n) {
    TailOperands t{0.f, 0.f, 0.f};
    if (p.bias) t.bias = p.bias[n];
    if (EPI == DGS_EPI_GATE_RESIDUAL) {
        t.resid = p.resid[(size_t)m * p.ldo + n];
        t.gate = p.gate[(size_t)(m / p.rows_per_batch) * p.gate_stride + n];
    }
    return t;
}
template <int EPI, class P>
__device__ __forceinline__ void tail_store(const P& p, int m, int n, float v, const TailOperands& t) {
    v += t.bias;
    const int b = m / p.rows_per_batch;
    const size_t o = (size_t)m * p.ldo + n;
    auto bf1 = [](float x) { return (bf16_t)(pack_bf2(x, 0.0f) & 0xffffu); };
    if (EPI == DGS_EPI_F32) { reinterpret_cast<float*>(p.out)[o] = v; return; }
    if (EPI == DGS_EPI_QKV) {
        const int third = p.N / 3;
        if (n >= 2 * third) p.vt[((size_t)b * third + (n - 2 * third)) * p.rows_per_batch + (m - b * p.rows_per_batch)] = bf1(v);
        else reinterpret_cast<bf16_t*>(p.out)[o] = bf1(n < third ? v * p.q_scale : v);
        return;
    }
    if (EPI == DGS_EPI_GATE_RESIDUAL) {
        reinterpret_cast<float*>(p.out)[o] = t.resid + t.gate * v;
        if (p.aux) reinterpret_cast<bf16_t*>(p.aux)[o] = bf1(v);
        return;
    }
    if (EPI == DGS_EPI_GELU_BF16) {
        if (p.aux) reinterpret_cast<bf16_t*>(p.aux)[o] = bf1(v);
        v = epi_gelu_tanh(v);
    } else if (EPI == DGS_EPI_DGELU_BF16) {
        v *= epi_dgelu_tanh(__uint_as_float((unsigned)reinterpret_cast<const bf16_t*>(p.aux)[o] << 16));
    }
    reinterpret_cast<bf16_t*>(p.out)[o] = bf1(v);
    if (p.vt) p.vt[((size_t)b * p.N + n) * p.rows_per_batch + (m - b * p.rows_per_batch)] = bf1(v);
}


}
```

### open-diffusiongs_amd/dgs_amd/_native.py

```python
import ctypes
import os

HERE = os.path.dirname(os.path.abspath(__file__))
LIB_PATH = os.environ.get("DGS_AMD_LIBRARY") or os.path.join(os.path.dirname(HERE), "lib", "libdgs_hip.so")

ABI_VERSION = 10
DGS_ERR_BINNING_OVERFLOW = -7
c_float_p = ctypes.POINTER(ctypes.c_float)
ALLOC_FN = ctypes.CFUNCTYPE(ctypes.c_void_p, ctypes.c_size_t, ctypes.c_void_p)


class DgsRasterForwardArgs(ctypes.Structure):
    _fields_ = [
        ("P", ctypes.c_int32), ("D", ctypes.c_int32), ("M", ctypes.c_int32),
        ("width", ctypes.c_int32), ("height", ctypes.c_int32), ("V", ctypes.c_int32), ("views_per_set", ctypes.c_int32),
        ("background", ctypes.c_void_p), ("means3D", ctypes.c_void_p), ("shs", ctypes.c_void_p),
        ("colors_precomp", ctypes.c_void_p), ("opacities", ctypes.c_void_p), ("scales", ctypes.c_void_p),
        ("rotations", ctypes.c_void_p), ("cov3D_precomp", ctypes.c_void_p), ("viewmatrix", ctypes.c_void_p),
        ("projmatrix", ctypes.c_void_p), ("campos", ctypes.c_void_p), ("tanfov", ctypes.c_void_p),
        ("tanfovx", ctypes.c_float), ("tanfovy", ctypes.c_float), ("scale_modifier", ctypes.c_float),
        ("prefiltered", ctypes.c_int32), ("debug", ctypes.c_int32), ("raw_activations", ctypes.c_int32),
        ("out_color", ctypes.c_void_p), ("radii", ctypes.c_void_p),
        ("geom_alloc", ALLOC_FN), ("geom_user", ctypes.c_void_p),
        ("img_alloc", ALLOC_FN), ("img_user", ctypes.c_void_p),
        ("binning_alloc", ALLOC_FN), ("binning_user", ctypes.c_void_p),
        ("binning_capacity", ctypes.c_int64), ("num_rendered_dev", ctypes.c_void_p), ("num_rendered_host", ctypes.c_void_p), ("longest_hint", ctypes.c_int64),
        ("num_rendered", ctypes.c_int64), ("longest_list", ctypes.c_int64), ("binning_form", ctypes.c_int32), ("exact_exp", ctypes.c_int32),
    ]


class DgsRasterBackwardArgs(ctypes.Structure):
    _fields_ = [
        ("P", ctypes.c_int32), ("D", ctypes.c_int32), ("M", ctypes.c_int32), ("width", ctypes.c_int32),
        ("height", ctypes.c_int32), ("V", ctypes.c_int32), ("views_per_set", ctypes.c_int32),
        ("num_rendered", ctypes.c_int64),
        ("background", ctypes.c_void_p), ("means3D", ctypes.c_void_p), ("shs", ctypes.c_void_p),
        ("colors_precomp", ctypes.c_void_p), ("opacities", ctypes.c_void_p), ("scales", ctypes.c_void_p),
        ("rotations", ctypes.c_void_p), ("cov3D_precomp", ctypes.c_void_p), ("viewmatrix", ctypes.c_void_p),
        ("projmatrix", ctypes.c_void_p), ("campos", ctypes.c_void_p), ("tanfov", ctypes.c_void_p),
        ("tanfovx", ctypes.c_float), ("tanfovy", ctypes.c_float), ("scale_modifier", ctypes.c_float),
        ("debug", ctypes.c_int32), ("raw_activations", ctypes.c_int32),
        ("radii", ctypes.c_void_p), ("dL_dpix", ctypes.c_void_p),
        ("geom_buffer", ctypes.c_void_p), ("binning_buffer", ctypes.c_void_p), ("img_buffer", ctypes.c_void_p),
        ("dL_dmeans2D", ctypes.c_void_p), ("dL_dconic", ctypes.c_void_p), ("dL_dcolors", ctypes.c_void_p),
        ("dL_dcov3D", ctypes.c_void_p), ("dL_dopacity", ctypes.c_void_p), ("dL_dmeans3D", ctypes.c_void_p),
        ("dL_dsh", ctypes.c_void_p), ("dL_dscales", ctypes.c_void_p), ("dL_drotations", ctypes.c_void_p),
        ("exact_exp", ctypes.c_int32), ("scratch", ctypes.c_void_p), ("scratch_bytes", ctypes.c_size_t),
    ]


RASTER_SYMBOLS = ["dgs_abi_version", "dgs_status_string", "dgs_raster_geom_bytes", "dgs_raster_image_bytes",
                  "dgs_raster_binning_bytes", "dgs_raster_forward", "dgs_raster_binning_form", "dgs_raster_backward",
                  "dgs_raster_backward_scratch_bytes", "dgs_mark_visible",
                  "dgs_raster_state_read", "dgs_cameras_from_c2w", "dgs_rays_from_c2w"]


def _declare(L):
    L.dgs_abi_version.restype = ctypes.c_int
    L.dgs_status_string.restype = ctypes.c_char_p
    L.dgs_status_string.argtypes = [ctypes.c_int]
    L.dgs_raster_geom_bytes.restype = ctypes.c_size_t
    L.dgs_raster_geom_bytes.argtypes = [ctypes.c_int32, ctypes.c_int32]
    L.dgs_raster_image_bytes.restype = ctypes.c_size_t
    L.dgs_raster_image_bytes.argtypes = [ctypes.c_int32, ctypes.c_int32, ctypes.c_int32]
    L.dgs_raster_binning_bytes.restype = ctypes.c_size_t
    L.dgs_raster_binning_bytes.argtypes = [ctypes.c_int64]
    L.dgs_raster_forward.restype = ctypes.c_int
    L.dgs_raster_forward.argtypes = [ctypes.POINTER(DgsRasterForwardArgs), ctypes.c_void_p]
    L.dgs_raster_binning_form.restype = ctypes.c_int
    L.dgs_raster_binning_form.argtypes = [ctypes.c_int32, ctypes.c_int64, ctypes.c_int64, ctypes.c_int32, ctypes.c_int32, ctypes.c_int32, ctypes.c_int32]
    if hasattr(L, "dgs_raster_backward"):
        L.dgs_raster_backward.restype = ctypes.c_int
        L.dgs_raster_backward.argtypes = [ctypes.POINTER(DgsRasterBackwardArgs), ctypes.c_void_p]
        L.dgs_raster_backward_scratch_bytes.restype = ctypes.c_size_t
        L.dgs_raster_backward_scratch_bytes.argtypes = [ctypes.c_int32, ctypes.c_int32, ctypes.c_int32, ctypes.c_int32, ctypes.c_int64]
    L.dgs_mark_visible.restype = ctypes.c_int
    L.dgs_mark_visible.argtypes = [ctypes.c_int32, ctypes.c_void_p, ctypes.c_void_p, ctypes.c_void_p, ctypes.c_void_p,
                                   ctypes.c_void_p]
    L.dgs_cameras_from_c2w.restype = ctypes.c_int
    L.dgs_cameras_from_c2w.argtypes = [ctypes.c_int32, ctypes.c_void_p, ctypes.c_void_p, ctypes.c_int32, ctypes.c_int32,
                                       ctypes.c_float, ctypes.c_float, ctypes.c_void_p, ctypes.c_void_p, ctypes.c_void_p,
                                       ctypes.c_void_p, ctypes.c_void_p]
    L.dgs_rays_from_c2w.restype = ctypes.c_int
    L.dgs_rays_from_c2w.argtypes = [ctypes.c_int32, ctypes.c_void_p, ctypes.c_void_p, ctypes.c_int32, ctypes.c_int32,
                                    ctypes.c_void_p, ctypes.c_void_p, ctypes.c_void_p]
    L.dgs_raster_state_read.restype = ctypes.c_int64
    L.dgs_raster_state_read.argtypes = [ctypes.c_char_p, ctypes.c_int32, ctypes.c_int32, ctypes.c_int32, ctypes.c_int32,
                                        ctypes.c_int64, ctypes.c_void_p, ctypes.c_void_p, ctypes.c_void_p, ctypes.c_void_p,
                                        ctypes.c_int64, ctypes.c_void_p]
    return L


def open_library(path):
    L = ctypes.CDLL(path)
    L.dgs_abi_version.restype = ctypes.c_int
    if L.dgs_abi_version() != ABI_VERSION:
        raise RuntimeError(f"dgs_amd: ABI version mismatch: {path} reports {L.dgs_abi_version()}, this binding is written for {ABI_VERSION} "
                           f"(include/dgs_raster.h DGS_ABI_VERSION) -- rebuild it (`python -m dgs_amd.build`, `DGS_INSTRUMENT=1 python -m dgs_amd.build`, "
                           f"tests/hipemu/build_emu.py)")
    return _declare(L)


_lib = None


def lib():
    global _lib
    if _lib is None:
        if not os.path.exists(LIB_PATH):
            raise RuntimeError(
                f"dgs_amd: HIP library {LIB_PATH} is missing. Build it with `python -m dgs_amd.build` "
                "(hipcc --offload-arch=gfx950). There is no CPU fallback.")
        import torch
        _lib = open_library(LIB_PATH)
        if _lib.dgs_abi_version() != ABI_VERSION:
            raise RuntimeError(f"dgs_amd: ABI version mismatch: libdgs_hip.so reports {_lib.dgs_abi_version()}, this binding is written "
                               f"for {ABI_VERSION} (include/dgs_raster.h DGS_ABI_VERSION) -- rebuild with `python -m dgs_amd.build`")
    return _lib


def status_string(L, code):
    return L.dgs_status_string(int(code)).decode()


EPI_BF16, EPI_GELU_BF16, EPI_GATE_RESIDUAL, EPI_F32, EPI_QKV, EPI_DGELU_BF16 = range(6)
GEMM_AUTO, GEMM_SIMPLE128, GEMM_SLICED, GEMM_QUAD, GEMM_SLICED128 = 0, 1, 4, 5, 6


class DgsDitGemmArgs(ctypes.Structure):
    _fields_ = [("M", ctypes.c_int32), ("N", ctypes.c_int32), ("K", ctypes.c_int32),
                ("A", ctypes.c_void_p), ("lda", ctypes.c_int32), ("W", ctypes.c_void_p), ("ldw", ctypes.c_int32),
                ("bias", ctypes.c_void_p), ("epilogue", ctypes.c_int32), ("out", ctypes.c_void_p), ("ldo", ctypes.c_int32),
                ("gate", ctypes.c_void_p), ("gate_stride", ctypes.c_int32), ("rows_per_batch", ctypes.c_int32),
                ("vt", ctypes.c_void_p), ("resid", ctypes.c_void_p), ("aux", ctypes.c_void_p), ("k_per_batch", ctypes.c_int32),
                ("a_batch_stride", ctypes.c_int64), ("w_batch_stride", ctypes.c_int64), ("algo", ctypes.c_int32),
                ("valid_rows", ctypes.c_int32), ("q_scale", ctypes.c_float), ("splitk_ws", ctypes.c_void_p)]


class DgsDitAttentionArgs(ctypes.Structure):
    _fields_ = [("B", ctypes.c_int32), ("heads", ctypes.c_int32), ("L", ctypes.c_int32), ("lpad", ctypes.c_int32),
                ("qk", ctypes.c_void_p), ("vt", ctypes.c_void_p), ("out", ctypes.c_void_p), ("scale", ctypes.c_float),
                ("ld_qk", ctypes.c_int32), ("k_offset", ctypes.c_int32), ("vt_batch_stride", ctypes.c_int64),
                ("lse2", ctypes.c_void_p), ("q_prescaled", ctypes.c_int32), ("tail_ws", ctypes.c_void_p),
                ("tail_ws_bytes", ctypes.c_size_t), ("tail_mode", ctypes.c_int32)]


class DgsDitAttentionBackwardArgs(ctypes.Structure):
    _fields_ = [("B", ctypes.c_int32), ("heads", ctypes.c_int32), ("L", ctypes.c_int32), ("lpad", ctypes.c_int32),
                ("qkv", ctypes.c_void_p), ("qkvT", ctypes.c_void_p), ("o", ctypes.c_void_p), ("dO", ctypes.c_void_p),
                ("dOT", ctypes.c_void_p), ("lse2", ctypes.c_void_p), ("D", ctypes.c_void_p), ("dqkv", ctypes.c_void_p),
                ("scale", ctypes.c_float), ("dqkvT", ctypes.c_void_p), ("bias_part", ctypes.c_void_p)]


class DgsDitLayerNormArgs(ctypes.Structure):
    _fields_ = [("rows", ctypes.c_int32), ("width", ctypes.c_int32), ("x", ctypes.c_void_p), ("weight", ctypes.c_void_p),
                ("shift", ctypes.c_void_p), ("scale", ctypes.c_void_p), ("mod_stride", ctypes.c_int32),
                ("rows_per_batch", ctypes.c_int32), ("eps", ctypes.c_float), ("out", ctypes.c_void_p),
                ("out_f32", ctypes.c_int32)]


class DgsDitRowLinearArgs(ctypes.Structure):
    _fields_ = [("M", ctypes.c_int32), ("N", ctypes.c_int32), ("K", ctypes.c_int32), ("x", ctypes.c_void_p),
                ("silu_input", ctypes.c_int32), ("W", ctypes.c_void_p), ("bias", ctypes.c_void_p),
                ("silu_output", ctypes.c_int32), ("out", ctypes.c_void_p)]


class DgsDitLayerNormBackwardArgs(ctypes.Structure):
    _fields_ = [("rows", ctypes.c_int32), ("width", ctypes.c_int32), ("x", ctypes.c_void_p), ("dh", ctypes.c_void_p),
                ("dh_f32", ctypes.c_int32), ("weight", ctypes.c_void_p), ("scale", ctypes.c_void_p),
                ("mod_stride", ctypes.c_int32), ("rows_per_batch", ctypes.c_int32), ("eps", ctypes.c_float),
                ("dx_in", ctypes.c_void_p), ("dx_out", ctypes.c_void_p), ("dshift", ctypes.c_void_p),
                ("dscale", ctypes.c_void_p), ("dweight", ctypes.c_void_p), ("scratch", ctypes.c_void_p), ("scratch_bytes", ctypes.c_size_t)]


class DgsDitRowLinearBackwardArgs(ctypes.Structure):
    _fields_ = [("M", ctypes.c_int32), ("N", ctypes.c_int32), ("K", ctypes.c_int32), ("x", ctypes.c_void_p),
                ("silu_input", ctypes.c_int32), ("W", ctypes.c_void_p), ("dy", ctypes.c_void_p), ("dW", ctypes.c_void_p),
                ("db", ctypes.c_void_p), ("dx", ctypes.c_void_p), ("scratch", ctypes.c_void_p), ("scratch_bytes", ctypes.c_size_t)]


class DgsDitGateMulArgs(ctypes.Structure):
    _fields_ = [("B", ctypes.c_int32), ("rows", ctypes.c_int32), ("width", ctypes.c_int32), ("dx", ctypes.c_void_p),
                ("y", ctypes.c_void_p), ("gate", ctypes.c_void_p), ("gate_stride", ctypes.c_int32), ("dy", ctypes.c_void_p),
                ("dyT", ctypes.c_void_p), ("dgate", ctypes.c_void_p), ("dbias", ctypes.c_void_p), ("scratch", ctypes.c_void_p),
                ("scratch_bytes", ctypes.c_size_t)]


class DgsDitLayerWeights(ctypes.Structure):
    _fields_ = [("qkv_w", ctypes.c_void_p), ("proj_w", ctypes.c_void_p), ("fc1_w", ctypes.c_void_p), ("fc2_w", ctypes.c_void_p),
                ("qkv_b", ctypes.c_void_p), ("proj_b", ctypes.c_void_p), ("fc1_b", ctypes.c_void_p), ("fc2_b", ctypes.c_void_p)]


class DgsDitModel(ctypes.Structure):
    _fields_ = [("width", ctypes.c_int32), ("heads", ctypes.c_int32), ("layers", ctypes.c_int32), ("patch", ctypes.c_int32),
                ("in_channels", ctypes.c_int32), ("n_gaussians", ctypes.c_int32), ("gs_channels", ctypes.c_int32),
                ("scene", ctypes.c_int32), ("relative_plk", ctypes.c_int32),
                ("range_near", ctypes.c_float), ("range_far", ctypes.c_float),
                ("t_w0", ctypes.c_void_p), ("t_b0", ctypes.c_void_p), ("t_w1", ctypes.c_void_p), ("t_b1", ctypes.c_void_p),
                ("tok_w", ctypes.c_void_p), ("pos_emb", ctypes.c_void_p), ("in_ln_w", ctypes.c_void_p),
                ("layer", ctypes.POINTER(DgsDitLayerWeights)),
                ("ada_w", ctypes.c_void_p), ("ada_b", ctypes.c_void_p),
                ("up_ln_w", ctypes.c_void_p), ("up_w", ctypes.c_void_p), ("dec_ln_w", ctypes.c_void_p), ("dec_w", ctypes.c_void_p)]


class DgsDitForwardArgs(ctypes.Structure):
    _fields_ = [("B", ctypes.c_int32), ("V", ctypes.c_int32), ("H", ctypes.c_int32), ("W", ctypes.c_int32),
                ("images", ctypes.c_void_p), ("ray_o", ctypes.c_void_p), ("ray_d", ctypes.c_void_p), ("t", ctypes.c_void_p),
                ("workspace", ctypes.c_void_p), ("workspace_bytes", ctypes.c_size_t),
                ("xyz", ctypes.c_void_p), ("features", ctypes.c_void_p), ("scaling", ctypes.c_void_p),
                ("rotation", ctypes.c_void_p), ("opacity", ctypes.c_void_p), ("aligned_xyz", ctypes.c_void_p),
                ("tokens", ctypes.c_void_p),
                ("prof_events", ctypes.POINTER(ctypes.c_void_p)), ("prof_kind", ctypes.c_int32),
                ("prof_capacity", ctypes.c_int32), ("prof_count", ctypes.POINTER(ctypes.c_int32)),
                ("train_recompute", ctypes.c_int32)]


class DgsDitLayerWeightsT(ctypes.Structure):
    _fields_ = [("qkv_wT", ctypes.c_void_p), ("proj_wT", ctypes.c_void_p), ("fc1_wT", ctypes.c_void_p), ("fc2_wT", ctypes.c_void_p)]


class DgsDitModelT(ctypes.Structure):
    _fields_ = [("layer", ctypes.POINTER(DgsDitLayerWeightsT)), ("dec_wT", ctypes.c_void_p)]


class DgsDitLayerGrads(ctypes.Structure):
    _fields_ = [(k, ctypes.c_void_p) for k in ("qkv_w", "proj_w", "fc1_w", "fc2_w", "qkv_b", "proj_b", "fc1_b", "fc2_b", "ada_w", "ada_b")]


class DgsDitGrads(ctypes.Structure):
    _fields_ = [(k, ctypes.c_void_p) for k in ("t_w0", "t_b0", "t_w1", "t_b1", "tok_w", "pos_emb", "in_ln_w")] + \
               [("layer", ctypes.POINTER(DgsDitLayerGrads))] + \
               [(k, ctypes.c_void_p) for k in ("head_ada_w", "head_ada_b", "up_ln_w", "up_w", "dec_ln_w", "dec_w")]


class DgsDitBackwardArgs(ctypes.Structure):
    _fields_ = [("B", ctypes.c_int32), ("V", ctypes.c_int32), ("H", ctypes.c_int32), ("W", ctypes.c_int32),
                ("ray_d", ctypes.c_void_p), ("saved", ctypes.c_void_p), ("saved_bytes", ctypes.c_size_t),
                ("workspace", ctypes.c_void_p), ("workspace_bytes", ctypes.c_size_t),
                ("dxyz", ctypes.c_void_p), ("dfeatures", ctypes.c_void_p), ("dscaling", ctypes.c_void_p),
                ("drotation", ctypes.c_void_p), ("dopacity", ctypes.c_void_p), ("recompute", ctypes.c_int32),
                ("block_done", ctypes.c_void_p), ("block_user", ctypes.c_void_p)]


BLOCK_DONE_FN = ctypes.CFUNCTYPE(None, ctypes.c_void_p, ctypes.c_int32)


class DgsDitRunBlocksArgs(ctypes.Structure):
    _fields_ = [("B", ctypes.c_int32), ("L", ctypes.c_int32), ("V", ctypes.c_int32), ("first", ctypes.c_int32), ("last", ctypes.c_int32),
                ("tokens_in", ctypes.c_void_p), ("cvec", ctypes.c_void_p), ("tokens_out", ctypes.c_void_p),
                ("workspace", ctypes.c_void_p), ("workspace_bytes", ctypes.c_size_t)]


DIT_SYMBOLS = ["dgs_dit_gemm", "dgs_dit_attention", "dgs_dit_attention_backward", "dgs_dit_layernorm_backward",
               "dgs_dit_rowlinear_backward", "dgs_dit_gate_mul", "dgs_dit_saved_bytes", "dgs_dit_backward_workspace_bytes",
               "dgs_dit_forward_train", "dgs_dit_backward", "dgs_dit_layernorm", "dgs_dit_rowlinear", "dgs_dit_lpad",
               "dgs_dit_workspace_bytes", "dgs_dit_forward", "dgs_dit_gemm_splitk_bytes",
               "dgs_dit_attention_tail_bytes", "dgs_dit_run_blocks", "dgs_debug_poison_lds", "dgs_debug_clock_probe",
               "dgs_dit_layernorm_backward_scratch_bytes", "dgs_dit_rowlinear_backward_scratch_bytes", "dgs_dit_gate_mul_scratch_bytes",
               "dgs_dit_workspace_bytes_for_tokens", "dgs_dit_attention_backward_slots", "dgs_dit_layernorm_gemm", "dgs_dit_layernorm_gemm_shares_rows", "dgs_dit_gemm_sliced_tile"]


def _declare_dit(L):
    L.dgs_dit_gemm_sliced_tile.restype = ctypes.c_int32
    L.dgs_dit_gemm_sliced_tile.argtypes = [ctypes.POINTER(DgsDitGemmArgs)]
    L.dgs_dit_layernorm_gemm_shares_rows.restype = ctypes.c_int32
    L.dgs_dit_layernorm_gemm_shares_rows.argtypes = [ctypes.POINTER(DgsDitLayerNormArgs), ctypes.POINTER(DgsDitGemmArgs)]
    L.dgs_dit_layernorm_gemm.restype = ctypes.c_int
    L.dgs_dit_layernorm_gemm.argtypes = [ctypes.POINTER(DgsDitLayerNormArgs), ctypes.POINTER(DgsDitGemmArgs), ctypes.c_void_p]
    L.dgs_dit_attention_backward_slots.restype = ctypes.c_int32
    L.dgs_dit_attention_backward_slots.argtypes = [ctypes.c_int32]
    for name, argt in (("dgs_dit_gemm", DgsDitGemmArgs), ("dgs_dit_attention", DgsDitAttentionArgs),
                       ("dgs_dit_attention_backward", DgsDitAttentionBackwardArgs),
                       ("dgs_dit_layernorm_backward", DgsDitLayerNormBackwardArgs),
                       ("dgs_dit_rowlinear_backward", DgsDitRowLinearBackwardArgs), ("dgs_dit_gate_mul", DgsDitGateMulArgs),
                       ("dgs_dit_layernorm", DgsDitLayerNormArgs), ("dgs_dit_rowlinear", DgsDitRowLinearArgs)):
        fn = getattr(L, name)
        fn.restype = ctypes.c_int
        fn.argtypes = [ctypes.POINTER(argt), ctypes.c_void_p]
    for fn in (L.dgs_dit_layernorm_backward_scratch_bytes, L.dgs_dit_rowlinear_backward_scratch_bytes, L.dgs_dit_gate_mul_scratch_bytes):
        fn.restype = ctypes.c_size_t
        fn.argtypes = [ctypes.c_int32] * 3
    L.dgs_dit_gemm_splitk_bytes.restype = ctypes.c_size_t
    L.dgs_dit_gemm_splitk_bytes.argtypes = [ctypes.c_int32] * 4
    L.dgs_dit_attention_tail_bytes.restype = ctypes.c_size_t
    L.dgs_dit_attention_tail_bytes.argtypes = [ctypes.c_int32] * 3
    L.dgs_dit_lpad.restype = ctypes.c_int32
    L.dgs_dit_lpad.argtypes = [ctypes.c_int32]
    L.dgs_dit_workspace_bytes.restype = ctypes.c_size_t
    L.dgs_dit_workspace_bytes.argtypes = [ctypes.POINTER(DgsDitModel), ctypes.c_int32, ctypes.c_int32, ctypes.c_int32, ctypes.c_int32]
    L.dgs_dit_workspace_bytes_for_tokens.restype = ctypes.c_size_t
    L.dgs_dit_workspace_bytes_for_tokens.argtypes = [ctypes.POINTER(DgsDitModel), ctypes.c_int32, ctypes.c_int32]
    for fn in (L.dgs_dit_saved_bytes, L.dgs_dit_backward_workspace_bytes):
        fn.restype = ctypes.c_size_t
        fn.argtypes = [ctypes.POINTER(DgsDitModel), ctypes.c_int32, ctypes.c_int32, ctypes.c_int32, ctypes.c_int32]
    L.dgs_dit_saved_bytes.argtypes = L.dgs_dit_saved_bytes.argtypes + [ctypes.c_int32]
    L.dgs_debug_poison_lds.restype = ctypes.c_int
    L.dgs_debug_poison_lds.argtypes = [ctypes.c_void_p]
    L.dgs_debug_clock_probe.restype = ctypes.c_int
    L.dgs_debug_clock_probe.argtypes = [ctypes.c_void_p, ctypes.c_int32, ctypes.c_void_p]
    L.dgs_dit_run_blocks.restype = ctypes.c_int
    L.dgs_dit_run_blocks.argtypes = [ctypes.POINTER(DgsDitModel), ctypes.POINTER(DgsDitRunBlocksArgs), ctypes.c_void_p]
    L.dgs_dit_forward_train.restype = ctypes.c_int
    L.dgs_dit_forward_train.argtypes = [ctypes.POINTER(DgsDitModel), ctypes.POINTER(DgsDitForwardArgs), ctypes.c_void_p,
                                        ctypes.c_size_t, ctypes.c_void_p]
    L.dgs_dit_backward.restype = ctypes.c_int
    L.dgs_dit_backward.argtypes = [ctypes.POINTER(DgsDitModel), ctypes.POINTER(DgsDitModelT), ctypes.POINTER(DgsDitGrads),
                                   ctypes.POINTER(DgsDitBackwardArgs), ctypes.c_void_p]
    L.dgs_dit_forward.restype = ctypes.c_int
    L.dgs_dit_forward.argtypes = [ctypes.POINTER(DgsDitModel), ctypes.POINTER(DgsDitForwardArgs), ctypes.c_void_p]
    return L


class DgsSamplerStepArgs(ctypes.Structure):
    _fields_ = [("B", ctypes.c_int32), ("per_sample", ctypes.c_int64), ("model_stride", ctypes.c_int64), ("model_offset", ctypes.c_int64),
                ("model_output", ctypes.c_void_p), ("x_t", ctypes.c_void_p), ("noise", ctypes.c_void_p), ("t", ctypes.c_void_p),
                ("coef1", ctypes.c_void_p), ("coef2", ctypes.c_void_p), ("sigma", ctypes.c_void_p), ("T", ctypes.c_int32),
                ("clip_denoised", ctypes.c_int32), ("out", ctypes.c_void_p), ("pred_xstart", ctypes.c_void_p), ("bad_t", ctypes.c_void_p)]


SAMPLER_SYMBOLS = ["dgs_sampler_step"]


def _declare_sampler(L):
    L.dgs_sampler_step.restype = ctypes.c_int
    L.dgs_sampler_step.argtypes = [ctypes.POINTER(DgsSamplerStepArgs), ctypes.c_void_p]
    return L


class DgsMseArgs(ctypes.Structure):
    _fields_ = [("B", ctypes.c_int32), ("n", ctypes.c_int64), ("rendering", ctypes.c_void_p), ("target", ctypes.c_void_p),
                ("clamp01", ctypes.c_int32), ("l2", ctypes.c_void_p), ("psnr", ctypes.c_void_p), ("grad", ctypes.c_void_p),
                ("grad_scale", ctypes.c_float), ("partial", ctypes.c_void_p)]


LOSS_CHUNKS = 64
class DgsResizeArgs(ctypes.Structure):
    _fields_ = [("planes", ctypes.c_int32), ("in_h", ctypes.c_int32), ("in_w", ctypes.c_int32), ("out_h", ctypes.c_int32),
                ("out_w", ctypes.c_int32), ("src", ctypes.c_void_p), ("dst", ctypes.c_void_p), ("mul", ctypes.c_float),
                ("add", ctypes.c_float), ("ddst", ctypes.c_void_p), ("dsrc", ctypes.c_void_p)]


class DgsPointsLossArgs(ctypes.Structure):
    _fields_ = [("B", ctypes.c_int32), ("V", ctypes.c_int32), ("H", ctypes.c_int32), ("W", ctypes.c_int32), ("aligned", ctypes.c_void_p),
                ("ray_o", ctypes.c_void_p), ("gt", ctypes.c_void_p), ("masks", ctypes.c_void_p), ("pointsdist", ctypes.c_void_p),
                ("xyz", ctypes.c_void_p), ("w_pointsdist", ctypes.c_void_p), ("w_xyz", ctypes.c_float), ("grad", ctypes.c_void_p),
                ("workspace", ctypes.c_void_p)]


class DgsSsimArgs(ctypes.Structure):
    _fields_ = [("N", ctypes.c_int32), ("C", ctypes.c_int32), ("H", ctypes.c_int32), ("W", ctypes.c_int32), ("B", ctypes.c_int32),
                ("x", ctypes.c_void_p), ("y", ctypes.c_void_p), ("data_range", ctypes.c_float), ("ssim", ctypes.c_void_p),
                ("l2", ctypes.c_void_p), ("psnr", ctypes.c_void_p), ("saved", ctypes.c_void_p), ("workspace", ctypes.c_void_p),
                ("g", ctypes.c_void_p), ("mse_scale", ctypes.c_void_p), ("dx", ctypes.c_void_p)]


LOSS_SYMBOLS = ["dgs_mse_psnr", "dgs_resize_bilinear", "dgs_resize_bilinear_backward", "dgs_points_loss", "dgs_points_loss_workspace_floats",
                "dgs_ssim", "dgs_ssim_backward", "dgs_ssim_workspace_floats", "dgs_ssim_saved_floats"]


def _declare_loss(L):
    L.dgs_mse_psnr.restype = ctypes.c_int
    L.dgs_mse_psnr.argtypes = [ctypes.POINTER(DgsMseArgs), ctypes.c_void_p]
    for fn in (L.dgs_resize_bilinear, L.dgs_resize_bilinear_backward):
        fn.restype = ctypes.c_int
        fn.argtypes = [ctypes.POINTER(DgsResizeArgs), ctypes.c_void_p]
    L.dgs_points_loss.restype = ctypes.c_int
    L.dgs_points_loss.argtypes = [ctypes.POINTER(DgsPointsLossArgs), ctypes.c_void_p]
    L.dgs_points_loss_workspace_floats.restype = ctypes.c_int64
    L.dgs_points_loss_workspace_floats.argtypes = [ctypes.c_int32, ctypes.c_int32]
    for fn in (L.dgs_ssim, L.dgs_ssim_backward):
        fn.restype = ctypes.c_int
        fn.argtypes = [ctypes.POINTER(DgsSsimArgs), ctypes.c_void_p]
    for fn in (L.dgs_ssim_workspace_floats, L.dgs_ssim_saved_floats):
        fn.restype = ctypes.c_int64
        fn.argtypes = [ctypes.c_int32] * 4
    return L


class DgsAdamWTensor(ctypes.Structure):
    _fields_ = [("p", ctypes.c_void_p), ("g", ctypes.c_void_p), ("m", ctypes.c_void_p), ("v", ctypes.c_void_p), ("copy", ctypes.c_void_p),
                ("copy_t", ctypes.c_void_p), ("rows", ctypes.c_int64), ("cols", ctypes.c_int64), ("copy_kind", ctypes.c_int32),
                ("first_tile", ctypes.c_int32)]


class DgsAdamWArgs(ctypes.Structure):
    _fields_ = [("tensors", ctypes.c_void_p), ("n_tensors", ctypes.c_int32), ("n_tiles", ctypes.c_int32), ("lr", ctypes.c_float),
                ("beta1", ctypes.c_float), ("beta2", ctypes.c_float), ("eps", ctypes.c_float), ("weight_decay", ctypes.c_float),
                ("bias_correction1", ctypes.c_float), ("bias_correction2_sqrt", ctypes.c_float),
                ("grad_sumsq", ctypes.c_void_p), ("max_grad_norm", ctypes.c_float)]


OPTIM_COPY_NONE, OPTIM_COPY_BF16, OPTIM_COPY_F32 = 0, 1, 2
OPTIM_SYMBOLS = ["dgs_adamw_plan", "dgs_adamw_step", "dgs_sumsq_count", "dgs_sumsq_partials", "dgs_sumsq_finish"]


def _declare_optim(L):
    L.dgs_adamw_plan.restype = ctypes.c_int32
    L.dgs_adamw_plan.argtypes = [ctypes.POINTER(DgsAdamWTensor), ctypes.c_int32]
    L.dgs_adamw_step.restype = ctypes.c_int
    L.dgs_adamw_step.argtypes = [ctypes.POINTER(DgsAdamWArgs), ctypes.c_void_p]
    L.dgs_sumsq_count.restype = ctypes.c_int32
    L.dgs_sumsq_count.argtypes = [ctypes.c_int64]
    L.dgs_sumsq_partials.restype = ctypes.c_int
    L.dgs_sumsq_partials.argtypes = [ctypes.c_void_p, ctypes.c_int64, ctypes.c_void_p, ctypes.c_void_p]
    L.dgs_sumsq_finish.restype = ctypes.c_int
    L.dgs_sumsq_finish.argtypes = [ctypes.c_void_p, ctypes.c_int32, ctypes.c_void_p, ctypes.c_void_p]
    return L


class DgsFieldArgs(ctypes.Structure):
    _fields_ = [("N", ctypes.c_int32), ("R", ctypes.c_int32), ("nb", ctypes.c_int32), ("split", ctypes.c_int32),
                ("xyz", ctypes.c_void_p), ("scaling", ctypes.c_void_p), ("rotation", ctypes.c_void_p), ("opacity", ctypes.c_void_p),
                ("mesh_scale", ctypes.c_float), ("scaling_modifier", ctypes.c_float), ("lin", ctypes.c_void_p), ("lo", ctypes.c_void_p),
                ("hi", ctypes.c_void_p), ("occ", ctypes.c_void_p), ("workspace", ctypes.c_void_p), ("workspace_bytes", ctypes.c_int64)]


FIELD_SYMBOLS = ["dgs_gaussian_field", "dgs_gaussian_field_workspace_bytes"]


def _declare_field(L):
    L.dgs_gaussian_field.restype = ctypes.c_int
    L.dgs_gaussian_field.argtypes = [ctypes.POINTER(DgsFieldArgs), ctypes.c_void_p]
    L.dgs_gaussian_field_workspace_bytes.restype = ctypes.c_int64
    L.dgs_gaussian_field_workspace_bytes.argtypes = [ctypes.c_int32, ctypes.c_int32]
    return L


class DgsEmaFusedArgs(ctypes.Structure):
    _fields_ = [("ema_base", ctypes.c_void_p), ("m_base", ctypes.c_void_p), ("one_minus_decay", ctypes.c_float)]


class DgsEmaTensor(ctypes.Structure):
    _fields_ = [("p", ctypes.c_void_p), ("ema", ctypes.c_void_p), ("copy", ctypes.c_void_p), ("copy_t", ctypes.c_void_p),
                ("rows", ctypes.c_int64), ("cols", ctypes.c_int64), ("copy_kind", ctypes.c_int32), ("first_tile", ctypes.c_int32)]


class DgsEmaArgs(ctypes.Structure):
    _fields_ = [("tensors", ctypes.c_void_p), ("n_tensors", ctypes.c_int32), ("n_tiles", ctypes.c_int32),
                ("one_minus_decay", ctypes.c_float), ("update", ctypes.c_int32), ("copy_source", ctypes.c_int32)]


EMA_SOURCE_NONE, EMA_SOURCE_P, EMA_SOURCE_EMA = 0, 1, 2
EMA_SYMBOLS = ["dgs_adamw_ema_step", "dgs_ema_plan", "dgs_ema_apply"]


def _declare_ema(L):
    L.dgs_adamw_ema_step.restype = ctypes.c_int
    L.dgs_adamw_ema_step.argtypes = [ctypes.POINTER(DgsAdamWArgs), ctypes.POINTER(DgsEmaFusedArgs), ctypes.c_void_p]
    L.dgs_ema_plan.restype = ctypes.c_int32
    L.dgs_ema_plan.argtypes = [ctypes.POINTER(DgsEmaTensor), ctypes.c_int32]
    L.dgs_ema_apply.restype = ctypes.c_int
    L.dgs_ema_apply.argtypes = [ctypes.POINTER(DgsEmaArgs), ctypes.c_void_p]
    return L


_declare_raster = _declare


def _declare(L):
    return _declare_ema(_declare_field(_declare_optim(_declare_loss(_declare_sampler(_declare_dit(_declare_raster(L)))))))
```

Baseline: 716.2 renders/s.

## Add 16x16x32 MFMA variant of sliced GEMM kernel, auto-enable for fc1 GELU

Adds an MS=16 template path to the sliced GEMM kernel that issues 16x16x32 bf16 MFMAs with its own fragment loads and f32x4 accumulators. It also adds an epilogue that relays the 16x16 accumulator layout through LDS into the existing strip store. Flag bits select the MFMA shape and tile width. By default the new path is used only for the fc1 GELU GEMM when M<=8192, aiming for better MFMA throughput or register use on that shape. The cost is extra LDS relayout work in the epilogue and a more complex fragment schedule.

Result: no change. 723.0 renders/s, median of 6 (+1.0%).

```diff
diff --git a/include/dgs_dit.h b/include/dgs_dit.h
--- a/include/dgs_dit.h
+++ b/include/dgs_dit.h
@@ -26,6 +26,11 @@
     DGS_GEMM_QUAD = 5,
     DGS_GEMM_SLICED128 = 6
 } DgsGemmAlgo;
+#define DGS_GEMM_ALGO_MASK 0xff
+#define DGS_GEMM_MFMA32 0x100
+#define DGS_GEMM_MFMA16 0x200
+#define DGS_GEMM_TILE256 0x400
+#define DGS_GEMM_TILE192 0x800
 
 typedef struct DgsDitGemmArgs {
     int32_t M, N, K;
diff --git a/open-diffusiongs_amd/csrc/dit_gemm.hip b/open-diffusiongs_amd/csrc/dit_gemm.hip
--- a/open-diffusiongs_amd/csrc/dit_gemm.hip
+++ b/open-diffusiongs_amd/csrc/dit_gemm.hip
@@ -261,8 +261,9 @@
     }
 }
 
-int sliced_gemm_tile(int M, int N, int K, int epilogue, int k_per_batch, int rows_per_batch, int valid_rows);
-int launch_sliced_gemm(const DgsDitGemmArgs* a, int bn, int rows_per_batch, int valid_rows, hipStream_t st, bool quad, bool rows_external);
+int sliced_gemm_tile(int M, int N, int K, int epilogue, int k_per_batch, int rows_per_batch, int valid_rows, int wide);
+int launch_sliced_gemm(const DgsDitGemmArgs* a, int bn, int rows_per_batch, int valid_rows, hipStream_t st, bool quad, bool rows_external, bool mfma16);
+bool sliced_mfma16_exists(int epilogue, int bn, bool quad);
 bool sliced_rows_are_gemv(int K, int N, int valid_rows);
 bool sliced128_eligible(int M, int N, int K, int epilogue, int k_per_batch, int rows_per_batch);
 int splitk_plan(int M, int N, int K, int k_per_batch, int* splits_per_batch);
@@ -271,6 +272,8 @@
 }
 
 using namespace dgs;
+
+static constexpr bool kAutoMfma16Fc1 = true, kAutoMfma16GateResidual = false, kAutoMfma16Qkv = false;
 
 template <int EPI>
 static void launch_gemm(const GemmParams& p0, int bn, hipStream_t st) {
@@ -315,20 +318,30 @@
     p.resid = a->resid ? a->resid : static_cast<const float*>(a->out);
     hipStream_t st0 = static_cast<hipStream_t>(stream);
     static const int env_algo = getenv("DGS_GEMM_ALGO") ? atoi(getenv("DGS_GEMM_ALGO")) : 0;
-    const int algo = a->algo ? a->algo : env_algo;
-    if (mode == 0 && (algo == DGS_GEMM_AUTO || algo == DGS_GEMM_SLICED) && a->splitk_ws && a->epilogue == DGS_EPI_F32 && !a->bias && a->ldo % 4 == 0 &&
+    const int algo = (a->algo & DGS_GEMM_ALGO_MASK) ? (a->algo & DGS_GEMM_ALGO_MASK) : env_algo;
+    static const int env_mfma = getenv("DGS_GEMM_MFMA") ? atoi(getenv("DGS_GEMM_MFMA")) : 0;
+    const int wide = (a->algo & DGS_GEMM_TILE256) ? 256 : (a->algo & DGS_GEMM_TILE192) ? 192 : 0;
+    const int force_mfma = (a->algo & DGS_GEMM_MFMA16) ? 16 : (a->algo & DGS_GEMM_MFMA32) ? 32 : 0;
+    if ((a->algo & DGS_GEMM_MFMA16) && (a->algo & DGS_GEMM_MFMA32)) return DGS_ERR_INVALID_ARGUMENT;
+    auto mfma16 = [&](int bn, bool quad) {
+        if (force_mfma) return force_mfma == 16;
+        if (!sliced_mfma16_exists(a->epilogue, bn, quad)) return false;
+        if (env_mfma) return env_mfma == 16;
+        return bn == 256 ? kAutoMfma16Fc1 && a->epilogue == DGS_EPI_GELU_BF16 && a->M <= 8192 : bn == 192 ? kAutoMfma16Qkv : kAutoMfma16GateResidual;
+    };
+    if (mode == 0 && force_mfma != 16 && (algo == DGS_GEMM_AUTO || algo == DGS_GEMM_SLICED) && a->splitk_ws && a->epilogue == DGS_EPI_F32 && !a->bias && a->ldo % 4 == 0 &&
         p.rows_per_batch == a->M && p.valid_rows == a->M) {
         int spb = 0;
         if (splitk_plan(a->M, a->N, a->K, kpb, &spb)) return launch_splitk_gemm(a, kpb, st0);
     }
-    const int sbn_auto = algo == DGS_GEMM_AUTO ? sliced_gemm_tile(a->M, a->N, a->K, a->epilogue, kpb, p.rows_per_batch, p.valid_rows) : 0;
+    const int sbn_auto = algo == DGS_GEMM_AUTO ? sliced_gemm_tile(a->M, a->N, a->K, a->epilogue, kpb, p.rows_per_batch, p.valid_rows, wide) : 0;
     const bool auto_sliced = sbn_auto != 0 && (a->M > 8192 || ((sbn_auto == 256 || sbn_auto == 192) && (a->epilogue == DGS_EPI_QKV ||
                                                                                   (a->epilogue == DGS_EPI_GELU_BF16 && a->N >= 4096))));
     if (algo == DGS_GEMM_SLICED || algo == DGS_GEMM_QUAD || auto_sliced) {
-        const int sbn = sliced_gemm_tile(a->M, a->N, a->K, a->epilogue, kpb, p.rows_per_batch, p.valid_rows);
+        const int sbn = sliced_gemm_tile(a->M, a->N, a->K, a->epilogue, kpb, p.rows_per_batch, p.valid_rows, wide);
         if (mode == 3) return sbn;
         if (mode == 2) return sbn && sliced_rows_are_gemv(a->K, a->N, p.valid_rows) && p.valid_rows < p.rows_per_batch ? 1 : 0;
-        if (sbn) return launch_sliced_gemm(a, sbn, p.rows_per_batch, p.valid_rows, st0, algo == DGS_GEMM_QUAD, mode == 1);
+        if (sbn) return launch_sliced_gemm(a, sbn, p.rows_per_batch, p.valid_rows, st0, algo == DGS_GEMM_QUAD, mode == 1, mfma16(sbn, algo == DGS_GEMM_QUAD));
     }
     if (mode == 2 || mode == 3) return 0;
     if (mode == 1) return DGS_ERR_INVALID_ARGUMENT;
@@ -337,7 +350,8 @@
     const bool few_tiles = (a->M / BM) * (a->N / 128) < 512 && a->N % 128 == 0;
     if ((algo == DGS_GEMM_SLICED128 || (algo == DGS_GEMM_AUTO && few_tiles && !no_s128 && a->K >= s128_mink)) &&
         sliced128_eligible(a->M, a->N, a->K, a->epilogue, kpb, p.rows_per_batch))
-        return launch_sliced_gemm(a, -128, p.rows_per_batch, p.valid_rows, st0, false, false);
+        return launch_sliced_gemm(a, -128, p.rows_per_batch, p.valid_rows, st0, false, false, mfma16(-128, false));
+    if (force_mfma == 16) return DGS_ERR_INVALID_ARGUMENT;
     if (a->epilogue == DGS_EPI_QKV && a->N % 128) return DGS_ERR_INVALID_ARGUMENT;
     static const int env_bn = getenv("DGS_GEMM_BN") ? atoi(getenv("DGS_GEMM_BN")) : 0;
     int bn = (a->N % 128 || ((a->M / BM) * (a->N / 128) < 512 && a->epilogue != DGS_EPI_QKV)) ? 64 : 128;
diff --git a/open-diffusiongs_amd/csrc/dit_gemm_deep.hip b/open-diffusiongs_amd/csrc/dit_gemm_deep.hip
--- a/open-diffusiongs_amd/csrc/dit_gemm_deep.hip
+++ b/open-diffusiongs_amd/csrc/dit_gemm_deep.hip
@@ -101,7 +101,7 @@
 __device__ long long dgs_gemm_dbg[16];
 __device__ unsigned dgs_gemm_tl[1024][4];
 
-template <int EPI, int BN, int NW, int EXP = 0, int BM = 256>
+template <int EPI, int BN, int NW, int EXP = 0, int BM = 256, int MS = 32>
 __global__ __launch_bounds__(NW == 8 ? 512 : 256) void gemm_sliced_kernel(DeepParams p) {
     constexpr int KW = (BM == 128 && NW == 8) ? 2 : 1, MW = NW / KW;
     constexpr int BK = 32, NS = (BM == 128 && KW == 1) ? 8 : 4;
@@ -115,6 +115,10 @@
     static_assert(NW == 8 || BN == 256 || (BM == 128 && BN == 128), "4 waves: 256 x 256 tiles (128 x 128 per wave) or 128 x 128 tiles (64 x 64)");
     static_assert(DUP == 0 || (DUP < NW && GW >= 1 && KW == 1), "a doubled piece only in the last W round");
     static_assert(WMB * NI >= G, "one DMA piece behind each MFMA of the spread half");
+    constexpr bool M16 = MS == 16;
+    constexpr int NA16 = 2 * WMB, NB16 = 2 * NI;
+    static_assert(MS == 32 || MS == 16, "MFMA shape: 32 (32x32x16) or 16 (16x16x32)");
+    static_assert(!M16 || (NW == 8 && EXP == 0 && NI >= 2), "16x16x32: the 8-wave forms");
     DGS_DYNAMIC_LDS(lds);
     const int dbg = kInstrumented ? p.dbg : 0;
     const long long dbg_k0 = dbg == 1 ? cycle_stamp() : 0;
@@ -223,20 +227,30 @@
     }
     const int tn = tile % p.tiles_n, rr = tile / p.tiles_n;
     const int m0 = ((rr / p.full_rows) * p.rows_ps + rr % p.full_rows) * BM, n0 = tn * BN;
-    f32x16 acc[WMB][NI];
-#pragma unroll
-    for (int i = 0; i < WMB; ++i)
-#pragma unroll
-        for (int j = 0; j < NI; ++j)
+    f32x16 acc[M16 ? 1 : WMB][M16 ? 1 : NI];
+    f32x4 acc16[M16 ? NA16 * NB16 : 1];
+#pragma unroll
+    for (int i = 0; i < (M16 ? 1 : WMB); ++i)
+#pragma unroll
+        for (int j = 0; j < (M16 ? 1 : NI); ++j)
 #pragma unroll
             for (int r = 0; r < 16; ++r) acc[i][j][r] = 0.0f;
-    int foff[2][NF];
+#pragma unroll
+    for (int q = 0; q < (M16 ? NA16 * NB16 : 1); ++q)
+#pragma unroll
+        for (int r = 0; r < 4; ++r) acc16[q][r] = 0.0f;
+    int foff[2][M16 ? 1 : NF];
 #pragma unroll
     for (int ks = 0; ks < 2; ++ks)
 #pragma unroll
-        for (int f = 0; f < NF; ++f)
+        for (int f = 0; f < (M16 ? 0 : NF); ++f)
             foff[ks][f] = kg * SUB + (f < WMB ? slab_off<BK>(wm * WROWS + 32 * f + frow, 2 * ks + fhalf) : A_BYTES + slab_off<BK>(wn * WN + 32 * (f - WMB) + frow, 2 * ks + fhalf));
     auto frag = [&](int slot, int ks, int f) { return *reinterpret_cast<const bf16x8*>(lds + slot * STAGE + foff[ks][f]); };
+    int foff16[M16 ? NA16 + NB16 : 1];
+#pragma unroll
+    for (int f = 0; f < (M16 ? NA16 + NB16 : 0); ++f)
+        foff16[f] = kg * SUB + (f < NA16 ? slab_off<BK>(wm * WROWS + 16 * f + (lane & 15), lane >> 4) : A_BYTES + slab_off<BK>(wn * WN + 16 * (f - NA16) + (lane & 15), lane >> 4));
+    auto frag16 = [&](int slot, int f) { return *reinterpret_cast<const bf16x8*>(lds + slot * STAGE + foff16[f]); };
     const int nk = p.K / (BK * KW);
     constexpr int GA = KW * A_BYTES / 1024 / NW;
     constexpr int RPI = 1024 / (2 * BK), CPR = BK / 8;
@@ -279,9 +293,17 @@
     if (has_side_job) sliced_for<2, NS - 1>([&](auto sc) { stage_next(sc); });
     wait_vmcnt<(NS - 3) * G>();
     raw_barrier();
-    bf16x8 fr[2][NF];
-#pragma unroll
-    for (int f = 0; f < NF; ++f) fr[0][f] = frag(0, 0, f);
+    bf16x8 fr[2][M16 ? 1 : NF];
+    bf16x8 fa[M16 ? NA16 : 1], fw[2][M16 ? NI : 1];
+    if constexpr (M16) {
+#pragma unroll
+        for (int a = 0; a < NA16; ++a) fa[a] = frag16(0, a);
+#pragma unroll
+        for (int w = 0; w < NI; ++w) fw[0][w] = frag16(0, NA16 + w);
+    } else {
+#pragma unroll
+        for (int f = 0; f < NF; ++f) fr[0][f] = frag(0, 0, f);
+    }
 
     long long dbg_wait = 0, dbg_bar = 0;
     constexpr bool SPREAD = NW == 4;
@@ -295,7 +317,19 @@
         constexpr int PRE_N = decltype(pre_tag)::value;
         constexpr bool refill = decltype(refill_tag)::value;
         if constexpr (refill && !SPREAD && EXP != 1) stage_next(SIC<(slot + NS - 1) % NS>{});
-        sliced_for<0, 2 * MF>([&](auto jc) {
+        if constexpr (M16) sliced_for<0, 4 * MF>([&](auto jc) {
+            constexpr int J = decltype(jc)::value, h = J / (2 * MF), f = J % (2 * MF), a = f / NI, w = f % NI;
+            constexpr int nslot = (slot + 1) % NS;
+            constexpr int c = a * NB16 + NI * h + w;
+            acc16[c] = __builtin_amdgcn_mfma_f32_16x16x32_bf16(fa[a], fw[h][w], acc16[c], 0, 0, 0);
+            sched_fence();
+            constexpr int STEP = (2 * MF - NA16) / NI, k = f - f / NI;
+            if constexpr (h == 0 && f % NA16 == 0 && f / NA16 < NI) fw[1][f / NA16] = frag16(slot, NA16 + NI + f / NA16);
+            else if constexpr (h == 1 && w == NI - 1) fa[a] = frag16(nslot, a);
+            else if constexpr (h == 1 && k % STEP == 0 && k / STEP < NI) fw[0][k / STEP] = frag16(nslot, NA16 + k / STEP);
+            sched_fence();
+        });
+        else sliced_for<0, 2 * MF>([&](auto jc) {
             constexpr int J = decltype(jc)::value, ks = J / MF, i = (J % MF) / NI, j = J % NI;
             acc[i][j] = __builtin_amdgcn_mfma_f32_32x32x16_bf16(fr[ks][i], fr[ks][WMB + j], acc[i][j], 0, 0, 0);
             sched_fence();
@@ -349,6 +383,11 @@
     }
     const long long dbg_t1 = dbg == 1 ? cycle_stamp() : 0;
     const long long dbg_w2 = dbg == 1 ? wall_stamp() : 0;
+    auto strip = [&](auto nbs_tag, int i, int j, int mb, int nb, char* patch, const auto&... pre_opt) {
+        constexpr int NBS = decltype(nbs_tag)::value;
+        if constexpr (M16) store_strip16<EPI, NBS, NB16>(p, &acc16[2 * i * NB16 + 2 * j], mb, nb, lane, patch, pre_opt...);
+        else store_strip<EPI, NBS>(p, &acc[i][j], mb, nb, lane, patch, pre_opt...);
+    };
     if constexpr (KW > 1) {
         float* const xch = reinterpret_cast<float*>(lds);
         auto region = [&](int owner) { return xch + ((wq * 2 + owner) * NI * 16) * 64 + lane; };
@@ -364,18 +403,32 @@
 #pragma unroll
                 for (int r = 0; r < 16; ++r) blk[j][r] += src[(j * 16 + r) * 64];
         };
-        if (kg == 0) give(acc[1], region(1)); else give(acc[0], region(0));
+        auto give16 = [&](int i, float* dst) {
+#pragma unroll
+            for (int q = 0; q < 2 * NB16; ++q)
+#pragma unroll
+                for (int r = 0; r < 4; ++r) dst[(q * 4 + r) * 64] = acc16[2 * i * NB16 + q][r];
+        };
+        auto take16 = [&](int i, const float* src) {
+#pragma unroll
+            for (int q = 0; q < 2 * NB16; ++q)
+#pragma unroll
+                for (int r = 0; r < 4; ++r) acc16[2 * i * NB16 + q][r] += src[(q * 4 + r) * 64];
+        };
+        if constexpr (M16) { if (kg == 0) give16(1, region(1)); else give16(0, region(0)); }
+        else { if (kg == 0) give(acc[1], region(1)); else give(acc[0], region(0)); }
         __syncthreads();
-        if (kg == 0) take(acc[0], region(0)); else take(acc[1], region(1));
+        if constexpr (M16) { if (kg == 0) take16(0, region(0)); else take16(1, region(1)); }
+        else { if (kg == 0) take(acc[0], region(0)); else take(acc[1], region(1)); }
         __syncthreads();
         char* patch = lds + wave * epi_strip_bytes(2);
         const int mb = m0 + wm * WROWS + 32 * kg, nb = n0 + wn * WN;
         if (kg == 0) {
-            if constexpr (PREFETCH_RESID) store_strip<EPI, 2>(p, &acc[0][0], mb, nb, lane, patch, pre[0]);
-            else store_strip<EPI, 2>(p, &acc[0][0], mb, nb, lane, patch);
+            if constexpr (PREFETCH_RESID) strip(SIC<2>{}, 0, 0, mb, nb, patch, pre[0]);
+            else strip(SIC<2>{}, 0, 0, mb, nb, patch);
         } else {
-            if constexpr (PREFETCH_RESID) store_strip<EPI, 2>(p, &acc[1][0], mb, nb, lane, patch, pre[0]);
-            else store_strip<EPI, 2>(p, &acc[1][0], mb, nb, lane, patch);
+            if constexpr (PREFETCH_RESID) strip(SIC<2>{}, 1, 0, mb, nb, patch, pre[0]);
+            else strip(SIC<2>{}, 1, 0, mb, nb, patch);
         }
     } else
     if (epi_staged<EPI>(p)) {
@@ -386,19 +439,19 @@
 #pragma unroll
             for (int i = 0; i < WMB; ++i) {
                 const int mb = m0 + wm * WROWS + 32 * i;
-                if (straddles) { store_strip<EPI, 1>(p, &acc[i][0], mb, nb, lane, patch); store_strip<EPI, 1>(p, &acc[i][1], mb, nb + 32, lane, patch); }
-                else store_strip<EPI, 2>(p, &acc[i][0], mb, nb, lane, patch);
-                store_strip<EPI, 1>(p, &acc[i][NI - 1], mb, nb + 32 * (NI - 1), lane, patch);
+                if (straddles) { strip(SIC<1>{}, i, 0, mb, nb, patch); strip(SIC<1>{}, i, 1, mb, nb + 32, patch); }
+                else strip(SIC<2>{}, i, 0, mb, nb, patch);
+                strip(SIC<1>{}, i, NI - 1, mb, nb + 32 * (NI - 1), patch);
             }
         } else
 #pragma unroll
         for (int i = 0; i < WMB; ++i)
 #pragma unroll
             for (int j = 0; j < NI; j += 2) {
-                if constexpr (PREFETCH_RESID) store_strip<EPI, 2>(p, &acc[i][j], m0 + wm * WROWS + 32 * i, n0 + wn * WN + 32 * j, lane, patch, pre[i * (NI / 2) + j / 2]);
-                else store_strip<EPI, 2>(p, &acc[i][j], m0 + wm * WROWS + 32 * i, n0 + wn * WN + 32 * j, lane, patch);
+                if constexpr (PREFETCH_RESID) strip(SIC<2>{}, i, j, m0 + wm * WROWS + 32 * i, n0 + wn * WN + 32 * j, patch, pre[i * (NI / 2) + j / 2]);
+                else strip(SIC<2>{}, i, j, m0 + wm * WROWS + 32 * i, n0 + wn * WN + 32 * j, patch);
             }
-    } else {
+    } else if constexpr (!M16) {
 #pragma unroll
         for (int i = 0; i < WMB; ++i) store_block<EPI, NI>(p, acc[i], m0 + wm * WROWS + 32 * i + 4 * fhalf, n0 + wn * WN, lane);
     }
@@ -422,7 +475,7 @@
     }
 }
 
-template <int EPI, int BN, int NW = 8, int BM = 256>
+template <int EPI, int BN, int NW = 8, int BM = 256, int MS = 32>
 static int launch_sliced(DeepParams p, hipStream_t st) {
     constexpr int LDS = (BM == 128 ? 8 : 4) * (BM * 32 * 2 + BN * 32 * 2);
     p.tiles_n = p.N / BN;
@@ -460,8 +513,8 @@
     const int rows_all = samples * p.full_rows;
     p.map2d = !no_map2d && BM == 256 && p.nsplit <= 1 && p.tail_wgs == 0 && rows_all % 4 == 0 && p.tiles_n % 2 == 0 && p.nfull_items % 8 == 0 &&
               p.nfull_items <= compute_unit_count_cached() ? 1 : 0;
-    auto kern = gemm_sliced_kernel<EPI, BN, NW, 0, BM>;
-    if constexpr (kInstrumented && EPI == DGS_EPI_F32 && BN == 256 && BM == 256) {
+    auto kern = gemm_sliced_kernel<EPI, BN, NW, 0, BM, MS>;
+    if constexpr (kInstrumented && EPI == DGS_EPI_F32 && BN == 256 && BM == 256 && MS == 32) {
         static const int exp = getenv("DGS_GEMM_EXP") ? atoi(getenv("DGS_GEMM_EXP")) : 0;
         if (exp == 1) kern = gemm_sliced_kernel<EPI, BN, NW, 1>;
         if (exp == 2) kern = gemm_sliced_kernel<EPI, BN, NW, 2>;
@@ -508,16 +561,18 @@
             for (int i = 0; i < nt; ++i) { if (p.tail_wgs == 0 && i < p.ntail) { se += (tl[i][1] - tl[i][0]) / 100.0; ++c1; } else { s2 += (tl[i][1] - tl[i][0]) / 100.0; ++c2; } }
             fprintf(stderr, "\n[gemm timeline] prologue us: %d workgroups with a side job %.2f, %d without %.2f\n", c1, c1 ? se / c1 : 0.0, c2, c2 ? s2 / c2 : 0.0);
         }
-        fprintf(stderr, "[gemm dbg] M=%d N=%d K=%d BN=%d: prologue %lld, loop %lld cycles (%lld per slab), vmcnt wait %lld, barrier %lld, epilogue %lld | slowest wg %lld cycles, max vmcnt wait %lld per slab, workgroup 0: %lld cycles in %.2f us = %.0f MHz\n", p.M,
-                p.N, p.K, BN, h[4], h[0], h[0] / h[3], h[1] / h[3], h[2] / h[3], h[5], h[6], h[7] / h[3], h[10], h[11] / 100.0, h[10] / (h[11] / 100.0));
+        fprintf(stderr, "[gemm dbg] M=%d N=%d K=%d BN=%d mfma=%s: prologue %lld, loop %lld cycles (%lld per slab), vmcnt wait %lld, barrier %lld, epilogue %lld | slowest wg %lld cycles, max vmcnt wait %lld per slab, workgroup 0: %lld cycles in %.2f us = %.0f MHz\n", p.M,
+                p.N, p.K, BN, MS == 16 ? "16x16x32" : "32x32x16", h[4], h[0], h[0] / h[3], h[1] / h[3], h[2] / h[3], h[5], h[6], h[7] / h[3], h[10], h[11] / 100.0, h[10] / (h[11] / 100.0));
     }
 #endif
     return hipGetLastError() == hipSuccess ? DGS_OK : DGS_ERR_DEVICE;
 }
 
-int sliced_gemm_tile(int M, int N, int K, int epilogue, int k_per_batch, int rows_per_batch, int valid_rows) {
+int sliced_gemm_tile(int M, int N, int K, int epilogue, int k_per_batch, int rows_per_batch, int valid_rows, int wide) {
     if (k_per_batch != K || K % 128 || M % 256 || rows_per_batch % 256) return 0;
     if (epilogue == DGS_EPI_QKV && N % 3) return 0;
+    if (wide == 256 && N % 256 == 0) return 256;
+    if (wide == 192 && N % 192 == 0 && epilogue == DGS_EPI_QKV) return 192;
     int full_rows = 0;
     for (int i = 0; i < rows_per_batch / 256; ++i)
         if ((valid_rows - i * 256 + 31) / 32 > 1) ++full_rows;
@@ -539,7 +594,14 @@
     return last_live <= 2 && K >= 512 && K <= 4096 && (K & (K - 1)) == 0 && N % 64 == 0;
 }
 
-int launch_sliced_gemm(const DgsDitGemmArgs* a, int bn, int rows_per_batch, int valid_rows, hipStream_t st, bool quad, bool rows_external) {
+bool sliced_mfma16_exists(int epilogue, int bn, bool quad) {
+    if (quad) return false;
+    if (bn == 256) return epilogue == DGS_EPI_GELU_BF16 || epilogue == DGS_EPI_F32;
+    if (bn == 192) return epilogue == DGS_EPI_QKV;
+    return bn == -128 && epilogue == DGS_EPI_GATE_RESIDUAL;
+}
+
+int launch_sliced_gemm(const DgsDitGemmArgs* a, int bn, int rows_per_batch, int valid_rows, hipStream_t st, bool quad, bool rows_external, bool mfma16) {
     DeepParams p;
     p.rows_external = rows_external ? 1 : 0;
     p.M = a->M; p.N = a->N; p.K = a->K; p.lda = a->lda; p.ldw = a->ldw; p.ldo = a->ldo; p.gate_stride = a->gate_stride;
@@ -551,6 +613,12 @@
     static const int s128_nw4 = getenv("DGS_GEMM_S128_NW4") ? atoi(getenv("DGS_GEMM_S128_NW4")) : 0;
 #define DGS_SLICED_CASE(E) case E: return bn == 256 ? (quad ? launch_sliced<E, 256, 4>(p, st) : launch_sliced<E, 256>(p, st)) : \
                                    bn == 128 ? launch_sliced<E, 128>(p, st) : s128_nw4 ? launch_sliced<E, 128, 4, 128>(p, st) : launch_sliced<E, 128, 8, 128>(p, st)
+    if (mfma16) {
+        if (!sliced_mfma16_exists(a->epilogue, bn, quad) || (bn == -128 && s128_nw4)) return DGS_ERR_INVALID_ARGUMENT;
+        if (bn == 192) return launch_sliced<DGS_EPI_QKV, 192, 8, 256, 16>(p, st);
+        if (bn == -128) return launch_sliced<DGS_EPI_GATE_RESIDUAL, 128, 8, 128, 16>(p, st);
+        return a->epilogue == DGS_EPI_F32 ? launch_sliced<DGS_EPI_F32, 256, 8, 256, 16>(p, st) : launch_sliced<DGS_EPI_GELU_BF16, 256, 8, 256, 16>(p, st);
+    }
     if (bn == 192) return a->epilogue == DGS_EPI_QKV && !quad ? launch_sliced<DGS_EPI_QKV, 192>(p, st) : DGS_ERR_INVALID_ARGUMENT;
     switch (a->epilogue) {
         DGS_SLICED_CASE(DGS_EPI_BF16);
diff --git a/open-diffusiongs_amd/csrc/dit_gemm_epilogue.h b/open-diffusiongs_amd/csrc/dit_gemm_epilogue.h
--- a/open-diffusiongs_amd/csrc/dit_gemm_epilogue.h
+++ b/open-diffusiongs_amd/csrc/dit_gemm_epilogue.h
@@ -62,12 +62,41 @@
     for (int it = 0; it < 32 / RPI; ++it) pre[it] = *reinterpret_cast<const float4*>(p.resid + (size_t)(m0 + it * RPI + rr) * p.ldo + n0 + cc);
 }
 
-template <int EPI, int NB, bool HAVE_PRE, class P>
-__device__ __forceinline__ void store_strip_impl(const P& p, const f32x16* acc, int m0, int n0, int lane, char* patch, const float4 (&pre)[4 * NB]) {
+struct Acc32 { const f32x16* a; };
+template <int PITCH> struct Acc16 { const f32x4* a; };
+template <class T> struct acc_is16 { static constexpr bool value = false; };
+template <int PITCH> __device__ __forceinline__ constexpr int acc_pitch(const Acc16<PITCH>&) { return PITCH; }
+template <int PITCH> struct acc_is16<Acc16<PITCH>> { static constexpr bool value = true; };
+
+template <int NB, int PITCH>
+__device__ __forceinline__ void relayout_16_to_32(const Acc16<PITCH>& acc, int lane, char* patch, f32x16 (&v)[NB]) {
+    constexpr int S = 32 * NB + 4;
+    float* st = reinterpret_cast<float*>(patch);
+    const int c16 = lane & 15, q = lane >> 4, c = lane & 31, half = lane >> 5;
+#pragma unroll
+    for (int rb = 0; rb < 2; ++rb)
+#pragma unroll
+        for (int cb = 0; cb < 2 * NB; ++cb)
+#pragma unroll
+            for (int r = 0; r < 4; ++r) st[(16 * rb + 4 * q + r) * S + 16 * cb + c16] = acc.a[rb * PITCH + cb][r];
+    __builtin_amdgcn_wave_barrier();
+#pragma unroll
+    for (int blk = 0; blk < NB; ++blk)
+#pragma unroll
+        for (int r = 0; r < 16; ++r) v[blk][r] = st[((r & 3) + 8 * (r >> 2) + 4 * half) * S + 32 * blk + c];
+    __builtin_amdgcn_wave_barrier();
+}
+
+template <int EPI, int NB, bool HAVE_PRE, class P, class ACC>
+__device__ __forceinline__ void store_strip_impl(const P& p, const ACC& accv, int m0, int n0, int lane, char* patch, const float4 (&pre)[4 * NB]) {
     constexpr int C = 32 * NB, S = C + 4;
+    constexpr bool A16 = acc_is16<ACC>::value;
     const int c = lane & 31, half = lane >> 5;
     const int b = m0 / p.rows_per_batch;
     if (EPI == DGS_EPI_QKV && n0 >= (p.N / 3) * 2) {
+        f32x16 v32[A16 ? NB : 1];
+        const f32x16* acc;
+        if constexpr (A16) { relayout_16_to_32<NB>(accv, lane, patch, v32); acc = v32; } else { (void)v32; acc = accv.a; }
 #pragma unroll
         for (int blk = 0; blk < NB; ++blk) {
             const int n = n0 + 32 * blk + c;
@@ -82,15 +111,33 @@
         return;
     }
     float* st = reinterpret_cast<float*>(patch);
-#pragma unroll
-    for (int blk = 0; blk < NB; ++blk) {
-        const int n = n0 + 32 * blk + c;
-        const float bias = p.bias ? p.bias[n] : 0.0f;
-        const float qs = (EPI == DGS_EPI_QKV && n < p.N / 3) ? p.q_scale : 1.0f;
-#pragma unroll
-        for (int r = 0; r < 16; ++r) {
-            const int row = (r & 3) + 8 * (r >> 2) + 4 * half;
-            st[row * S + 32 * blk + c] = EPI == DGS_EPI_QKV ? (acc[blk][r] + bias) * qs : acc[blk][r] + bias;
+    if constexpr (A16) {
+        const int c16 = lane & 15, q4 = lane >> 4;
+#pragma unroll
+        for (int cb = 0; cb < 2 * NB; ++cb) {
+            const int n = n0 + 16 * cb + c16;
+            const float bias = p.bias ? p.bias[n] : 0.0f;
+            const float qs = (EPI == DGS_EPI_QKV && n < p.N / 3) ? p.q_scale : 1.0f;
+#pragma unroll
+            for (int rb = 0; rb < 2; ++rb)
+#pragma unroll
+                for (int r = 0; r < 4; ++r) {
+                    const float a = accv.a[rb * acc_pitch(accv) + cb][r];
+                    st[(16 * rb + 4 * q4 + r) * S + 16 * cb + c16] = EPI == DGS_EPI_QKV ? (a + bias) * qs : a + bias;
+                }
+        }
+    } else {
+        const f32x16* acc = accv.a;
+#pragma unroll
+        for (int blk = 0; blk < NB; ++blk) {
+            const int n = n0 + 32 * blk + c;
+            const float bias = p.bias ? p.bias[n] : 0.0f;
+            const float qs = (EPI == DGS_EPI_QKV && n < p.N / 3) ? p.q_scale : 1.0f;
+#pragma unroll
+            for (int r = 0; r < 16; ++r) {
+                const int row = (r & 3) + 8 * (r >> 2) + 4 * half;
+                st[row * S + 32 * blk + c] = EPI == DGS_EPI_QKV ? (acc[blk][r] + bias) * qs : acc[blk][r] + bias;
+            }
         }
     }
     __builtin_amdgcn_wave_barrier();
@@ -162,11 +209,20 @@
 template <int EPI, int NB, class P>
 __device__ __forceinline__ void store_strip(const P& p, const f32x16* acc, int m0, int n0, int lane, char* patch) {
     const float4 none[4 * NB] = {};
-    store_strip_impl<EPI, NB, false>(p, acc, m0, n0, lane, patch, none);
+    store_strip_impl<EPI, NB, false>(p, Acc32{acc}, m0, n0, lane, patch, none);
 }
 template <int EPI, int NB, class P>
 __device__ __forceinline__ void store_strip(const P& p, const f32x16* acc, int m0, int n0, int lane, char* patch, const float4 (&pre)[4 * NB]) {
-    store_strip_impl<EPI, NB, true>(p, acc, m0, n0, lane, patch, pre);
+    store_strip_impl<EPI, NB, true>(p, Acc32{acc}, m0, n0, lane, patch, pre);
+}
+template <int EPI, int NB, int PITCH, class P>
+__device__ __forceinline__ void store_strip16(const P& p, const f32x4* acc, int m0, int n0, int lane, char* patch) {
+    const float4 none[4 * NB] = {};
+    store_strip_impl<EPI, NB, false>(p, Acc16<PITCH>{acc}, m0, n0, lane, patch, none);
+}
+template <int EPI, int NB, int PITCH, class P>
+__device__ __forceinline__ void store_strip16(const P& p, const f32x4* acc, int m0, int n0, int lane, char* patch, const float4 (&pre)[4 * NB]) {
+    store_strip_impl<EPI, NB, true>(p, Acc16<PITCH>{acc}, m0, n0, lane, patch, pre);
 }
 
 struct TailOperands { float bias, resid, gate; };
diff --git a/open-diffusiongs_amd/dgs_amd/_native.py b/open-diffusiongs_amd/dgs_amd/_native.py
--- a/open-diffusiongs_amd/dgs_amd/_native.py
+++ b/open-diffusiongs_amd/dgs_amd/_native.py
@@ -125,6 +125,8 @@
 
 EPI_BF16, EPI_GELU_BF16, EPI_GATE_RESIDUAL, EPI_F32, EPI_QKV, EPI_DGELU_BF16 = range(6)
 GEMM_AUTO, GEMM_SIMPLE128, GEMM_SLICED, GEMM_QUAD, GEMM_SLICED128 = 0, 1, 4, 5, 6
+GEMM_MFMA32, GEMM_MFMA16 = 0x100, 0x200
+GEMM_TILE256, GEMM_TILE192 = 0x400, 0x800
 
 
 class DgsDitGemmArgs(ctypes.Structure):
```
